# ruiguo-bio/smer_music_generation

Hardware: AMD Instinct MI355X
Metric: infill tokens/sec + train tokens/sec, SMER seq_len=1024, 1/2/4/8 MI355X (higher is better)
Workload: dtype bf16; 1 GPU; C2 train step: 6+6 layers d512 h8 ff2048 V309, per-GPU B=32 S=1024 T=256, dropout 0.1, fused WCE + Adam; global_batch=32, seq_len=1024, tgt_len=256, parallelism=dp1

## Files before the change

include/smer_hip.h:

```cpp
#ifndef SMER_HIP_H
#define SMER_HIP_H

#include <stddef.h>
#include <stdint.h>

#ifdef __cplusplus
extern "C" {
#endif

typedef struct ihipStream_t* smer_stream_t;

#define SMER_OK 0
#define SMER_ERR_INVALID (-1)
#define SMER_ERR_HIP (-2)
#define SMER_ERR_UNSUPPORTED (-3)

#define SMER_F32 0
#define SMER_BF16 1

int smer_abi_version(void);
const char* smer_last_error(void);

int smer_gemm(int dtype, int a_kcontig, int b_kcontig, int M, int N, int K,
              const void* A, long lda, const void* B, long ldb,
              const float* bias, float alpha, int relu,
              const void* residual, long ldr,
              const void* gate, long ldg, float gate_scale,
              float drop_p, uint32_t drop_seed,
              void* C, long ldc, float* Cf, long ldcf, int accumulate,
              void* workspace, size_t ws_bytes, smer_stream_t stream);

int smer_gemm_wgrad_bias(int dtype, int M, int N, int K, const void* dy, long lddy,
                         const void* x, long ldx, float* dW, long lddw, int accumulate,
                         float* db, int db_accumulate, void* workspace, size_t ws_bytes,
                         smer_stream_t stream);
int smer_gemm_wgrad_bias_ex(int dtype, int M, int N, int K, const void* dy, long lddy,
                            const void* x, long ldx, float* dW, long lddw, int accumulate,
                            float* db, int db_accumulate, void* workspace, size_t ws_bytes,
                            int max_workgroups, smer_stream_t stream);
int smer_gemm_wgrad_fp8(int M, int N, int K, const void* dy8, long lddy, const void* x8, long ldx,
                        const float* dy_inv, const float* x_inv, float* dW, long lddw, int accumulate,
                        float* db, int db_accumulate, void* workspace, size_t ws_bytes,
                        int max_workgroups, smer_stream_t stream);

int smer_gemm_debug_stamps(void* buf, size_t bytes);

int smer_attn_drop_mask_gen(int B, int H, int Lq, int Lk, float drop_p, uint32_t seed, void* mask,
                            smer_stream_t stream);
int smer_attn_fwd(int dtype, int B, int H, int Lq, int Lk, int D,
                  const void* q, long ldq, const void* k, long ldk, const void* v, long ldv,
                  void* o, long ldo, float* lse, const uint8_t* kpm, int causal, float scale,
                  float drop_p, uint32_t seed, void* drop_mask, int drop_mask_in,
                  smer_stream_t stream);
size_t smer_attn_drop_mask_bytes(int B, int H, int Lq, int Lk);
size_t smer_attn_bwd_workspace(int dtype, int B, int H, int Lq, int Lk);
int smer_attn_bwd(int dtype, int B, int H, int Lq, int Lk, int D,
                  const void* q, long ldq, const void* k, long ldk, const void* v, long ldv,
                  const void* o, long ldo, const void* dout, long lddo, const float* lse,
                  const uint8_t* kpm, int causal, float scale, float drop_p, uint32_t seed,
                  void* dq, long lddq, void* dk, long lddk, void* dv, long lddv,
                  void* workspace, size_t ws_bytes, const void* drop_mask,
                  smer_stream_t stream);
int smer_attn_bwd_fp8(int B, int H, int Lq, int Lk, int D, const void* q, long ldq,
                      const void* k, long ldk, const void* v, long ldv, const void* o, long ldo,
                      const void* dout, long lddo, const float* lse, const uint8_t* kpm,
                      int causal, float scale, float drop_p, uint32_t seed, void* dq, long lddq,
                      void* dk, long lddk, void* dv, long lddv, void* workspace, size_t ws_bytes,
                      const void* drop_mask, void* dq8, long lddq8, void* dk8, long lddk8,
                      void* dv8, long lddv8, const float* qs, unsigned* amax, smer_stream_t stream);
int smer_attn_fwd_fp8(int B, int H, int Lq, int Lk, int D, const void* q, long ldq, const void* k,
                      long ldk, const void* v, long ldv, void* o, long ldo, float* lse,
                      const uint8_t* kpm, int causal, float scale, float drop_p, uint32_t seed,
                      void* drop_mask, int drop_mask_in, void* o8, long ldo8, const float* qs,
                      unsigned* amax, smer_stream_t stream);
int smer_attn_weights(int dtype, int B, int H, int Lq, int Lk, int D,
                      const void* q, long ldq, const void* k, long ldk, const float* lse,
                      const uint8_t* kpm, int causal, float scale, float* out,
                      smer_stream_t stream);
int smer_attn_decode(int dtype, int n_rows, int H, int D, const void* q, long ldq,
                     const void* kcache, const void* vcache, long row_stride, long req_stride,
                     long head_stride, const int32_t* row_req, const int32_t* row_nkeys,
                     void* o, long ldo, float scale, smer_stream_t stream);
int smer_kv_scatter_heads(int dtype, int n_rows, int H, int D, const void* src, long lds,
                          void* cache, long req_stride, long kv_stride, long head_stride,
                          const int32_t* row_req, const int32_t* row_pos, smer_stream_t stream);
int smer_kv_scatter(int dtype, int n_rows, int width, const void* src, long lds,
                    void* cache, long row_stride, long req_stride,
                    const int32_t* row_req, const int32_t* row_pos, smer_stream_t stream);
int smer_linear_decode(int M, int N, int K, const void* A, long lda, const void* W, long ldw,
                       const float* bias, int relu, const void* residual, long ldr, void* C,
                       long ldc, float* Cf, long ldcf, void* kv, long kv_row_stride,
                       long kv_req_stride, const int32_t* kv_req, const int32_t* kv_pos,
                       int kv_col0, smer_stream_t stream);
int smer_attn_decode_qln(int n_rows, int H, int D, const void* y, long ldy, const float* gamma,
                         const float* beta, float eps, const void* wq, long ldw, const float* bq,
                         void* x_out, long ldx, int dmodel, const void* kcache, const void* vcache,
                         long row_stride, long req_stride, long head_stride, const int32_t* row_req,
                         const int32_t* row_nkeys, void* o, long ldo, float scale,
                         smer_stream_t stream);
int smer_attn_decode_shared(int dtype, int n_rows, int H, int D, const void* q, long ldq,
                            const void* kcache, const void* vcache, long row_stride,
                            long req_stride, long head_stride, const int32_t* row_req,
                            const int32_t* row_nkeys, const int32_t* group_tab, int n_groups,
                            void* o, long ldo, float scale, smer_stream_t stream);
int smer_attn_decode_shared_qln(int n_rows, int H, int D, const void* y, long ldy,
                                const float* gamma, const float* beta, float eps, const void* wq,
                                long ldw, const float* bq, void* x_out, long ldx, int dmodel,
                                const void* kcache, const void* vcache, long row_stride,
                                long req_stride, long head_stride, const int32_t* row_req,
                                const int32_t* row_nkeys, const int32_t* group_tab, int n_groups,
                                void* o, long ldo, float scale, smer_stream_t stream);
int smer_linear_decode_ln(int M, int N, int K, const void* Y, long ldy, const float* gamma,
                          const float* beta, float eps, void* X, long ldx, const void* W, long ldw,
                          const float* bias, int relu, const void* residual, long ldr, void* C,
                          long ldc, float* Cf, long ldcf, void* kv, long kv_row_stride,
                          long kv_req_stride, const int32_t* kv_req, const int32_t* kv_pos,
                          int kv_col0, smer_stream_t stream);
int smer_linear_decode_f32(int M, int N, int K, const void* A, long lda, const void* W, long ldw,
                           const float* bias, int relu, const void* residual, long ldr, void* C,
                           long ldc, float* Cf, long ldcf, void* kv, long kv_row_stride,
                           long kv_req_stride, const int32_t* kv_req, const int32_t* kv_pos,
                           int kv_col0, smer_stream_t stream);
int smer_linear_decode_ln_f32(int M, int N, int K, const void* Y, long ldy, const float* gamma,
                              const float* beta, float eps, void* X, long ldx, const void* W,
                              long ldw, const float* bias, int relu, const void* residual,
                              long ldr, void* C, long ldc, float* Cf, long ldcf, void* kv,
                              long kv_row_stride, long kv_req_stride, const int32_t* kv_req,
                              const int32_t* kv_pos, int kv_col0, smer_stream_t stream);
int smer_attn_decode_split_f32(int n_rows, int H, int D, const void* q, long ldq, const void* kcache,
                               const void* vcache, long row_stride, long req_stride, long head_stride,
                               const int32_t* row_req, const int32_t* row_nkeys, float* part, float scale,
                               smer_stream_t stream);
int smer_attn_decode_split_qln_f32(int n_rows, int H, int D, const float* y, long ldy, const float* gamma,
                                   const float* beta, float eps, const float* wq, long ldw, const float* bq,
                                   float* x_out, long ldx, int dmodel, const void* kcache, const void* vcache,
                                   long row_stride, long req_stride, long head_stride, const int32_t* row_req,
                                   const int32_t* row_nkeys, float* part, float scale, smer_stream_t stream);
int smer_linear_decode_merge_f32(int M, int N, int K, const float* part, const void* W, long ldw,
                                 const float* bias, int relu, const void* residual, long ldr, void* C,
                                 long ldc, float* Cf, long ldcf, smer_stream_t stream);
int smer_grammar_greedy_step(int R, int V, const float* logits, long ldl, int32_t* state,
                             int nst, const int8_t* targets, int max_masks, const uint8_t* keep,
                             const uint8_t* cls, int eos, int m0, int trash_pos, int max_span,
                             const int32_t* src_len, int64_t* ids, int32_t* meta,
                             int32_t* out_tok, int cap, int32_t* alive, smer_stream_t stream);
int smer_grammar_greedy_step_ring(int R, int V, const float* logits, long ldl, int32_t* state,
                                  int nst, const int8_t* targets, int max_masks,
                                  const uint8_t* keep, const uint8_t* cls, int eos, int m0,
                                  int trash_pos, int max_span, const int32_t* src_len,
                                  int64_t* ids, int32_t* meta, int32_t* out_tok, int cap,
                                  int32_t* ctl, int32_t* ring, int ring_n, smer_stream_t stream);
int smer_grammar_sample_step(int R, int V, const float* logits, long ldl, int32_t* state, int nst,
                             const int8_t* targets, int max_masks, const uint8_t* keep,
                             const uint8_t* reject, const uint8_t* cls, int eos, int m0,
                             int trash_pos, int max_span, const int32_t* src_len, int64_t* ids,
                             int32_t* meta, int32_t* out_tok, int cap, uint32_t* mt, int32_t* ctl,
                             int32_t* ring, int ring_n, smer_stream_t stream);
int smer_grammar_sample_step_tp(int R, int V, const float* logits, long ldl, int32_t* state, int nst,
                                const int8_t* targets, int max_masks, const uint8_t* keep,
                                const uint8_t* reject, const uint8_t* cls, int eos, int m0,
                                int trash_pos, int max_span, const int32_t* src_len, int64_t* ids,
                                int32_t* meta, int32_t* out_tok, int cap, uint32_t* mt, int32_t* ctl,
                                int32_t* ring, int ring_n, const double* tp, smer_stream_t stream);
int smer_grammar_sample_step_rows(int R, int V, const float* logits, long ldl, int32_t* state, int nst,
                                  const int8_t* targets, int max_masks, const uint8_t* keep,
                                  const uint8_t* reject, const uint8_t* cls, int eos, int m0,
                                  int trash_pos, int max_span, const int32_t* src_len, int64_t* ids,
                                  int32_t* meta, int32_t* out_tok, int cap, uint32_t* mt, long ldmt,
                                  int32_t* ctl, int32_t* ring, int ring_n, const double* tp,
                                  smer_stream_t stream);

int smer_layernorm_fwd(int dtype, int M, int N, const void* x, long ldx,
                       const float* gamma, const float* beta, float eps,
                       void* y, long ldy, float* mean, float* rstd, smer_stream_t stream);
size_t smer_layernorm_bwd_workspace(int M, int N);
int smer_layernorm_bwd(int dtype, int M, int N, const void* dy, long lddy, int dy_f32,
                       const void* x, long ldx, const float* mean, const float* rstd,
                       const float* gamma, void* dx, long lddx,
                       void* dx_drop, long ldxd, float drop_p, uint32_t seed,
                       float* dgamma, float* dbeta, int accumulate,
                       void* workspace, size_t ws_bytes, smer_stream_t stream);
int smer_layernorm_bwd_partials(int dtype, int M, int N, const void* dy, long lddy, int dy_f32,
                                const void* x, long ldx, const float* mean, const float* rstd,
                                const float* gamma, void* dx, long lddx, void* dx_drop,
                                long ldxd, float drop_p, uint32_t seed, void* workspace,
                                size_t ws_bytes, smer_stream_t stream);
int smer_layernorm_param_reduce(int M, int N, void* workspace, size_t ws_bytes, float* dgamma,
                                float* dbeta, int accumulate, smer_stream_t stream);

int smer_embed_fwd(int dtype, int n_tok, int d, const int64_t* ids, const int32_t* positions,
                   int L, const float* table, const float* pe, float scale,
                   float drop_p, uint32_t seed, void* out, long ldo, smer_stream_t stream);
int smer_embed_fwd_fp8(int n_tok, int d, const int64_t* ids, const int32_t* positions, int L,
                       const float* table, const float* pe, float scale, float drop_p, uint32_t seed,
                       void* out, long ldo, void* q8, long ldq, const float* qs, unsigned* amax,
                       smer_stream_t stream);
size_t smer_embed_bwd_workspace(int V, int d, int n_tok_total);
int smer_embed_bwd(int dtype, int V, int d, float scale,
                   const int64_t* ids0, const void* dx0, long ld0, int n0, float p0, uint32_t seed0,
                   const int64_t* ids1, const void* dx1, long ld1, int n1, float p1, uint32_t seed1,
                   float* dtable, void* workspace, size_t ws_bytes, smer_stream_t stream);

int smer_wce_denom(int n, const int64_t* y, const float* ce_all, float* denom,
                   smer_stream_t stream);
int smer_wce_fwd_bwd(int dtype, int R, int V, const float* logits, long ldl, const int64_t* y,
                     const float* w, const float* denom, float* row_loss, float* loss_out,
                     void* dlogits, long ldd, float grad_scale, smer_stream_t stream);

int smer_adam(long n, float* p, const float* g, float* m, float* v, void* p_bf16,
              float lr, float b1, float b2, float eps, float bc1, float bc2_sqrt,
              smer_stream_t stream);

int smer_cast(int src_dtype, int dst_dtype, long n, const void* src, void* dst,
              smer_stream_t stream);
int smer_cast2d(int src_dtype, int dst_dtype, int rows, int cols, const void* src, long lds,
                void* dst, long ldd, smer_stream_t stream);
int smer_debug_checksum(const void* p, long rows, long row_bytes, long ld_bytes,
                        unsigned long long* out, int nparts, smer_stream_t stream);
int smer_argmax_accuracy(int R, int V, const float* logits, long ldl, const int64_t* y,
                         const int32_t* cls, int ncls, int pad, unsigned* counts,
                         smer_stream_t stream);
size_t smer_colsum_workspace(int M, int N);
int smer_colsum(int dtype, int M, int N, const void* x, long ldx, float* out, int accumulate,
                void* workspace, size_t ws_bytes, smer_stream_t stream);

size_t smer_fp8_quantize_workspace(void);
int smer_fp8_quantize(int rows, int cols, const void* x, long ldx, void* q, long ldq,
                      void* workspace, float* inv_scale, smer_stream_t stream);
int smer_fp8_quantize_segments(int nseg, const int64_t* seg, unsigned* amax_ws, float* inv_scale,
                               int blocks_per_seg, smer_stream_t stream);
int smer_gemm_fp8(int M, int N, int K, const void* A, long lda, const void* B, long ldb,
                  const float* a_inv, const float* b_inv, const float* bias, int relu,
                  const void* residual, long ldr, float drop_p, uint32_t drop_seed, void* C,
                  long ldc, smer_stream_t stream);

int smer_gemm_fp8_q(int M, int N, int K, const void* A, long lda, const void* B, long ldb,
                    const float* a_inv, const float* b_inv, const float* bias, int relu,
                    const void* residual, long ldr, float drop_p, uint32_t drop_seed, void* C,
                    long ldc, void* q8, long ldq8, const float* qs, unsigned* amax,
                    smer_stream_t stream);
int smer_layernorm_fwd_fp8(int M, int N, const void* x, long ldx, const float* gamma,
                           const float* beta, float eps, void* y, long ldy, float* mean,
                           float* rstd, void* q8, long ldq, const float* qs, unsigned* amax,
                           smer_stream_t stream);
int smer_fp8_scales(int n, const unsigned* amax_prev, float* qs, float* inv, unsigned* amax_next,
                    smer_stream_t stream);

int smer_fp8_quantize_segments_t(int nseg, const int64_t* seg, unsigned* amax_ws, float* inv_scale,
                                 int blocks_per_seg, smer_stream_t stream);
int smer_gemm_fp8_ex(int M, int N, int K, const void* A, long lda, const void* B, long ldb,
                     const float* a_inv, const float* b_inv, const float* bias, int relu,
                     const void* residual, long ldr, const void* gate, long ldg, float gate_scale,
                     float drop_p, uint32_t drop_seed, void* C, long ldc, void* q8, long ldq8,
                     const float* qs, unsigned* amax, smer_stream_t stream);
int smer_gemm_fp8_gate8(int M, int N, int K, const void* A, long lda, const void* B, long ldb,
                        const float* a_inv, const float* b_inv, const void* gate8, long ldg,
                        float gate_scale, void* C, long ldc, void* q8, long ldq8, const float* q8_scale,
                        unsigned* q8_amax, smer_stream_t stream);
int smer_layernorm_bwd_fp8(int M, int N, const void* dy, long lddy, const void* x, long ldx,
                           const float* mean, const float* rstd, const float* gamma, void* dx,
                           long lddx, void* dx_drop, long ldxd, float drop_p, uint32_t seed,
                           void* q8, long ldq, const float* qs, unsigned* amax, float* dgamma,
                           float* dbeta, int accumulate, void* workspace, size_t ws_bytes,
                           int partials_only, smer_stream_t stream);

#ifdef __cplusplus
}
#endif
#endif
```

smer_music_generation_amd/_lib.py:

```python
from __future__ import annotations

import ctypes
import os

import torch

_HERE = os.path.dirname(os.path.abspath(__file__))
LIB_PATH = os.environ.get("SMER_HIP_LIB") or os.path.join(_HERE, "libsmer_hip.so")

c_int, c_long, c_float, c_size, c_u32 = (ctypes.c_int, ctypes.c_long, ctypes.c_float,
                                         ctypes.c_size_t, ctypes.c_uint32)
P = ctypes.c_void_p

SIGNATURES = {
    "smer_abi_version": (c_int, []),
    "smer_last_error": (ctypes.c_char_p, []),
    "smer_gemm": (c_int, [c_int, c_int, c_int, c_int, c_int, c_int, P, c_long, P, c_long, P,
                          c_float, c_int, P, c_long, P, c_long, c_float, c_float, c_u32, P,
                          c_long, P, c_long, c_int, P, c_size, P]),
    "smer_gemm_debug_stamps": (c_int, [P, c_size]),
    "smer_gemm_wgrad_bias": (c_int, [c_int, c_int, c_int, c_int, P, c_long, P, c_long, P, c_long,
                                     c_int, P, c_int, P, c_size, P]),
    "smer_embed_fwd_fp8": (c_int, [c_int, c_int, P, P, c_int, P, P, c_float, c_float, c_u32, P, c_long, P, c_long,
                                   P, P, P]),
    "smer_gemm_wgrad_fp8": (c_int, [c_int, c_int, c_int, P, c_long, P, c_long, P, P, P, c_long, c_int, P, c_int,
                                    P, c_size, c_int, P]),
    "smer_gemm_wgrad_bias_ex": (c_int, [c_int, c_int, c_int, c_int, P, c_long, P, c_long, P, c_long,
                                        c_int, P, c_int, P, c_size, c_int, P]),
    "smer_attn_fwd": (c_int, [c_int, c_int, c_int, c_int, c_int, c_int, P, c_long, P, c_long, P,
                              c_long, P, c_long, P, P, c_int, c_float, c_float, c_u32, P, c_int, P]),
    "smer_attn_fwd_fp8": (c_int, [c_int, c_int, c_int, c_int, c_int, P, c_long, P, c_long, P, c_long,
                                  P, c_long, P, P, c_int, c_float, c_float, c_u32, P, c_int, P, c_long,
                                  P, P, P]),
    "smer_attn_drop_mask_gen": (c_int, [c_int, c_int, c_int, c_int, c_float, c_u32, P, P]),
    "smer_attn_drop_mask_bytes": (c_size, [c_int, c_int, c_int, c_int]),
    "smer_attn_bwd_workspace": (c_size, [c_int, c_int, c_int, c_int, c_int]),
    "smer_attn_bwd": (c_int, [c_int, c_int, c_int, c_int, c_int, c_int, P, c_long, P, c_long, P,
                              c_long, P, c_long, P, c_long, P, P, c_int, c_float, c_float, c_u32,
                              P, c_long, P, c_long, P, c_long, P, c_size, P, P]),
    "smer_attn_bwd_fp8": (c_int, [c_int, c_int, c_int, c_int, c_int, P, c_long, P, c_long, P, c_long,
                                  P, c_long, P, c_long, P, P, c_int, c_float, c_float, c_u32, P, c_long,
                                  P, c_long, P, c_long, P, c_size, P, P, c_long, P, c_long, P, c_long,
                                  P, P, P]),
    "smer_attn_weights": (c_int, [c_int, c_int, c_int, c_int, c_int, c_int, P, c_long, P, c_long,
                                  P, P, c_int, c_float, P, P]),
    "smer_attn_decode": (c_int, [c_int, c_int, c_int, c_int, P, c_long, P, P, c_long, c_long,
                                 c_long, P, P, P, c_long, c_float, P]),
    "smer_attn_decode_qln": (c_int, [c_int, c_int, c_int, P, c_long, P, P, c_float, P, c_long, P,
                                     P, c_long, c_int, P, P, c_long, c_long, c_long, P, P, P, c_long,
                                     c_float, P]),
    "smer_attn_decode_shared": (c_int, [c_int, c_int, c_int, c_int, P, c_long, P, P, c_long, c_long,
                                        c_long, P, P, P, c_int, P, c_long, c_float, P]),
    "smer_attn_decode_shared_qln": (c_int, [c_int, c_int, c_int, P, c_long, P, P, c_float, P, c_long,
                                            P, P, c_long, c_int, P, P, c_long, c_long, c_long, P, P,
                                            P, c_int, P, c_long, c_float, P]),
    "smer_kv_scatter_heads": (c_int, [c_int, c_int, c_int, c_int, P, c_long, P, c_long, c_long,
                                      c_long, P, P, P]),
    "smer_kv_scatter": (c_int, [c_int, c_int, c_int, P, c_long, P, c_long, c_long, P, P, P]),
    "smer_linear_decode": (c_int, [c_int, c_int, c_int, P, c_long, P, c_long, P, c_int, P, c_long,
                                   P, c_long, P, c_long, P, c_long, c_long, P, P, c_int, P]),
    "smer_linear_decode_ln": (c_int, [c_int, c_int, c_int, P, c_long, P, P, c_float, P, c_long, P,
                                      c_long, P, c_int, P, c_long, P, c_long, P, c_long, P, c_long,
                                      c_long, P, P, c_int, P]),
    "smer_linear_decode_f32": (c_int, [c_int, c_int, c_int, P, c_long, P, c_long, P, c_int, P, c_long,
                                       P, c_long, P, c_long, P, c_long, c_long, P, P, c_int, P]),
    "smer_linear_decode_ln_f32": (c_int, [c_int, c_int, c_int, P, c_long, P, P, c_float, P, c_long, P,
                                          c_long, P, c_int, P, c_long, P, c_long, P, c_long, P, c_long,
                                          c_long, P, P, c_int, P]),
    "smer_attn_decode_split_f32": (c_int, [c_int, c_int, c_int, P, c_long, P, P, c_long, c_long, c_long, P, P, P,
                                           c_float, P]),
    "smer_attn_decode_split_qln_f32": (c_int, [c_int, c_int, c_int, P, c_long, P, P, c_float, P, c_long, P, P,
                                               c_long, c_int, P, P, c_long, c_long, c_long, P, P, P, c_float, P]),
    "smer_linear_decode_merge_f32": (c_int, [c_int, c_int, c_int, P, P, c_long, P, c_int, P, c_long, P, c_long, P,
                                             c_long, P]),
    "smer_fp8_quantize_workspace": (c_size, []),
    "smer_fp8_quantize": (c_int, [c_int, c_int, P, c_long, P, c_long, P, P, P]),
    "smer_fp8_quantize_segments": (c_int, [c_int, P, P, P, c_int, P]),
    "smer_gemm_fp8": (c_int, [c_int, c_int, c_int, P, c_long, P, c_long, P, P, P, c_int, P, c_long,
                              c_float, c_u32, P, c_long, P]),
    "smer_gemm_fp8_q": (c_int, [c_int, c_int, c_int, P, c_long, P, c_long, P, P, P, c_int, P,
                                c_long, c_float, c_u32, P, c_long, P, c_long, P, P, P]),
    "smer_layernorm_fwd_fp8": (c_int, [c_int, c_int, P, c_long, P, P, c_float, P, c_long, P, P, P,
                                       c_long, P, P, P]),
    "smer_fp8_scales": (c_int, [c_int, P, P, P, P, P]),
    "smer_fp8_quantize_segments_t": (c_int, [c_int, P, P, P, c_int, P]),
    "smer_gemm_fp8_ex": (c_int, [c_int, c_int, c_int, P, c_long, P, c_long, P, P, P, c_int, P, c_long,
                                 P, c_long, c_float, c_float, c_u32, P, c_long, P, c_long, P, P, P]),
    "smer_gemm_fp8_gate8": (c_int, [c_int, c_int, c_int, P, c_long, P, c_long, P, P, P, c_long, c_float,
                                    P, c_long, P, c_long, P, P, P]),
    "smer_layernorm_bwd_fp8": (c_int, [c_int, c_int, P, c_long, P, c_long, P, P, P, P, c_long, P, c_long,
                                       c_float, c_u32, P, c_long, P, P, P, P, c_int, P, c_size, c_int,
                                       P]),
    "smer_grammar_greedy_step": (c_int, [c_int, c_int, P, c_long, P, c_int, P, c_int, P, P, c_int,
                                         c_int, c_int, c_int, P, P, P, P, c_int, P, P]),
    "smer_grammar_greedy_step_ring": (c_int, [c_int, c_int, P, c_long, P, c_int, P, c_int, P, P,
                                              c_int, c_int, c_int, c_int, P, P, P, P, c_int, P, P,
                                              c_int, P]),
    "smer_grammar_sample_step": (c_int, [c_int, c_int, P, c_long, P, c_int, P, c_int, P, P, P,
                                         c_int, c_int, c_int, c_int, P, P, P, P, c_int, P, P, P,
                                         c_int, P]),
    "smer_grammar_sample_step_tp": (c_int, [c_int, c_int, P, c_long, P, c_int, P, c_int, P, P, P,
                                            c_int, c_int, c_int, c_int, P, P, P, P, c_int, P, P, P,
                                            c_int, P, P]),
    "smer_grammar_sample_step_rows": (c_int, [c_int, c_int, P, c_long, P, c_int, P, c_int, P, P, P,
                                              c_int, c_int, c_int, c_int, P, P, P, P, c_int, P, c_long,
                                              P, P, c_int, P, P]),
    "smer_layernorm_fwd": (c_int, [c_int, c_int, c_int, P, c_long, P, P, c_float, P, c_long, P,
                                   P, P]),
    "smer_layernorm_bwd_workspace": (c_size, [c_int, c_int]),
    "smer_layernorm_bwd": (c_int, [c_int, c_int, c_int, P, c_long, c_int, P, c_long, P, P, P, P,
                                   c_long, P, c_long, c_float, c_u32, P, P, c_int, P, c_size, P]),
    "smer_layernorm_bwd_partials": (c_int, [c_int, c_int, c_int, P, c_long, c_int, P, c_long, P, P,
                                            P, P, c_long, P, c_long, c_float, c_u32, P, c_size, P]),
    "smer_layernorm_param_reduce": (c_int, [c_int, c_int, P, c_size, P, P, c_int, P]),
    "smer_embed_fwd": (c_int, [c_int, c_int, c_int, P, P, c_int, P, P, c_float, c_float, c_u32,
                               P, c_long, P]),
    "smer_embed_bwd_workspace": (c_size, [c_int, c_int, c_int]),
    "smer_embed_bwd": (c_int, [c_int, c_int, c_int, c_float, P, P, c_long, c_int, c_float, c_u32,
                               P, P, c_long, c_int, c_float, c_u32, P, P, c_size, P]),
    "smer_wce_denom": (c_int, [c_int, P, P, P, P]),
    "smer_wce_fwd_bwd": (c_int, [c_int, c_int, c_int, P, c_long, P, P, P, P, P, P, c_long,
                                 c_float, P]),
    "smer_adam": (c_int, [c_long, P, P, P, P, P, c_float, c_float, c_float, c_float, c_float,
                          c_float, P]),
    "smer_cast": (c_int, [c_int, c_int, c_long, P, P, P]),
    "smer_cast2d": (c_int, [c_int, c_int, c_int, c_int, P, c_long, P, c_long, P]),
    "smer_colsum_workspace": (c_size, [c_int, c_int]),
    "smer_colsum": (c_int, [c_int, c_int, c_int, P, c_long, P, c_int, P, c_size, P]),
    "smer_debug_checksum": (c_int, [P, c_long, c_long, c_long, P, c_int, P]),
    "smer_argmax_accuracy": (c_int, [c_int, c_int, P, c_long, P, P, c_int, c_int, P, P]),
}

_lib = None
_load_error = None


def load():
    global _lib, _load_error
    if _lib is not None:
        return _lib
    if not os.path.exists(LIB_PATH):
        _load_error = "libsmer_hip.so not built (%s); run __graft_entry__.build()" % LIB_PATH
        raise RuntimeError(_load_error)
    lib = ctypes.CDLL(LIB_PATH, mode=ctypes.RTLD_GLOBAL)
    for name, (res, args) in SIGNATURES.items():
        fn = getattr(lib, name)
        fn.restype = res
        fn.argtypes = args
    _lib = lib
    return lib


class SmerError(RuntimeError):
    pass


def check(status, what):
    if status != 0:
        msg = load().smer_last_error()
        raise SmerError("%s failed (%d): %s" % (what, status, msg.decode() if msg else ""))


def call(name, *args):
    lib = load()
    check(getattr(lib, name)(*args), name)
```

smer_music_generation_amd/csrc/common.h:

```cpp
#pragma once
#include <hip/hip_runtime.h>
#include <stdint.h>

#include "../../include/smer_hip.h"

typedef __bf16 bf16;
typedef __bf16 bf16x8 __attribute__((ext_vector_type(8)));
typedef __bf16 bf16x4 __attribute__((ext_vector_type(4)));
typedef short i16x4 __attribute__((ext_vector_type(4)));
typedef float f32x4 __attribute__((ext_vector_type(4)));

#define SMER_WAVE 64

extern "C" int smer_set_error(int code, const char* msg);
#define SMER_CHECK_LAUNCH(what)                                          \
  do {                                                                   \
    hipError_t _e = hipGetLastError();                                   \
    if (_e != hipSuccess) return smer_set_error(SMER_ERR_HIP, hipGetErrorString(_e)); \
  } while (0)
#define SMER_REQUIRE(cond, msg) \
  do { if (!(cond)) return smer_set_error(SMER_ERR_INVALID, msg); } while (0)

template <typename T> __device__ __forceinline__ float to_f32(T x);
template <> __device__ __forceinline__ float to_f32<float>(float x) { return x; }
// ... 11 lines not shown
    case 0x141: return __int_as_float(__builtin_amdgcn_mov_dpp(__float_as_int(v), 0x141, 0xF, 0xF, false));
    default: return __int_as_float(__builtin_amdgcn_mov_dpp(__float_as_int(v), 0x140, 0xF, 0xF, false));
  }
}
template <typename OP>
__device__ __forceinline__ float wave_reduce(float v, OP op) {
  v = op(v, dpp_f(v, 0xB1));
  v = op(v, dpp_f(v, 0x4E));
  v = op(v, dpp_f(v, 0x141));
  v = op(v, dpp_f(v, 0x140));
  const auto a = __builtin_amdgcn_permlane16_swap(__float_as_uint(v), __float_as_uint(v), false, false);
  v = op(__uint_as_float(a[0]), __uint_as_float(a[1]));
  const auto b = __builtin_amdgcn_permlane32_swap(__float_as_uint(v), __float_as_uint(v), false, false);
  return op(__uint_as_float(b[0]), __uint_as_float(b[1]));
}
__device__ __forceinline__ float wave_sum(float v) {
  return wave_reduce(v, [](float x, float y) { return x + y; });
}
__device__ __forceinline__ float wave_max(float v) {
  return wave_reduce(v, [](float x, float y) { return fmaxf(x, y); });
}

__device__ __forceinline__ uint32_t smer_mix32(uint32_t h) {
  h ^= h >> 16; h *= 0x7FEB352Du; h ^= h >> 15; h *= 0x846CA68Bu; h ^= h >> 16;
  return h;
}
__device__ __forceinline__ uint32_t smer_rowkey(uint32_t seed, uint32_t row) {
  return smer_mix32(smer_mix32(row ^ 0x85EBCA6Bu) ^ seed);
}
__device__ __forceinline__ uint32_t smer_pair_bits(uint32_t rowkey, uint32_t pair) {
  return smer_mix32(rowkey + pair * 0x9E3779B9u);
}
__device__ __forceinline__ bool smer_keep16(uint32_t rowkey, uint32_t thr16, uint32_t col) {
  const uint32_t h = smer_pair_bits(rowkey, col >> 1);
  return ((col & 1u) ? (h >> 16) : (h & 0xFFFFu)) >= thr16;
}
__device__ __forceinline__ void smer_drop8(uint32_t rowkey, uint32_t thr16, float ds, uint32_t col0,
                                           float (&v)[8]) {
#pragma unroll
  for (int k = 0; k < 4; ++k) {
    const uint32_t h = smer_pair_bits(rowkey, (col0 >> 1) + k);
    v[2 * k] = (h & 0xFFFFu) >= thr16 ? v[2 * k] * ds : 0.f;
    v[2 * k + 1] = (h >> 16) >= thr16 ? v[2 * k + 1] * ds : 0.f;
  }
}
static inline uint32_t smer_drop_thr16(float p) {
  if (p <= 0.f) return 0u;
  long t = (long)((double)p * 65536.0 + 0.5);
  return (uint32_t)(t < 1 ? 1 : (t > 65535 ? 65535 : t));
}
static inline float smer_drop_scale16(uint32_t thr16) {
  return thr16 ? (float)(65536.0 / (65536.0 - (double)thr16)) : 1.f;
}

__device__ __forceinline__ uint32_t smer_attn_bits(uint32_t rowkey, uint32_t quad) {
  uint32_t h = rowkey + quad * 0x9E3779B9u;
  h ^= h >> 16;
  h = __umul24(h, 0xEB352Du);
  h ^= h >> 15;
  h = __umul24(h, 0x6CA68Bu);
  h ^= h >> 16;
  return h;
}
__device__ __forceinline__ uint32_t smer_attn_ge(uint32_t h, uint32_t lo4) {
  return (h | 0x80808080u) - lo4;
}
__device__ __forceinline__ bool smer_attn_keep(uint32_t rowkey, uint32_t thr7, uint32_t key) {
  return ((smer_attn_bits(rowkey, key >> 2) >> (8 * (key & 3))) & 0x7Fu) >= thr7;
}
static inline uint32_t smer_attn_thr7(float p) {
  if (p <= 0.f) return 0u;
  long t = (long)((double)p * 128.0 + 0.5);
  return (uint32_t)(t < 1 ? 1 : (t > 127 ? 127 : t));
}
static inline float smer_attn_scale7(uint32_t thr7) {
  return thr7 ? (float)(128.0 / (128.0 - (double)thr7)) : 1.f;
}

size_t smer_col_reduce_scratch(int nblk, int N);
void smer_col_reduce_launch(int nblk, int N, const float* part, long stride, long off, float* out,
                            int accumulate, float scale, float* scratch, hipStream_t s,
                            float* out2 = nullptr, int nsplit = 0);

template <typename T, bool VEC = true>
__device__ __forceinline__ void load8(const T* p, int valid, float (&v)[8]) {
  if (VEC && valid >= 8) {
    if constexpr (sizeof(T) == 2) {
      bf16x8 r = *reinterpret_cast<const bf16x8*>(p);
#pragma unroll
      for (int i = 0; i < 8; ++i) v[i] = (float)r[i];
    } else {
      float4 a = *reinterpret_cast<const float4*>(p), b = *reinterpret_cast<const float4*>(p + 4);
      v[0] = a.x; v[1] = a.y; v[2] = a.z; v[3] = a.w; v[4] = b.x; v[5] = b.y; v[6] = b.z; v[7] = b.w;
    }
  } else {
#pragma unroll
    for (int i = 0; i < 8; ++i) v[i] = i < valid ? (float)p[i] : 0.f;
  }
}

constexpr int LNR_MAXC = 4;
template <int NC = LNR_MAXC>
__device__ __forceinline__ void ln_stats_loaded(const float (&v)[NC][8], int N, float eps, int lane, float& mu,
                                                float& rs) {
  const int nch = N >> 3;
  float s = 0.f;
#pragma unroll
  for (int c = 0; c < NC; ++c)
    if (lane + 64 * c < nch)
#pragma unroll
      for (int i = 0; i < 8; ++i) s += v[c][i];
  mu = wave_sum(s) / N;
  float q = 0.f;
#pragma unroll
  for (int c = 0; c < NC; ++c)
    if (lane + 64 * c < nch)
#pragma unroll
      for (int i = 0; i < 8; ++i) {
        const float d = v[c][i] - mu;
        q += d * d;
      }
  rs = rsqrtf(wave_sum(q) / N + eps);
}
template <typename T, int NC = LNR_MAXC>
__device__ __forceinline__ void ln_row_stats(const T* __restrict__ xr, int N, float eps, int lane,
                                             float (&v)[NC][8], float& mu, float& rs) {
  const int nch = N >> 3;
  float s = 0.f;
#pragma unroll
  for (int c = 0; c < NC; ++c) {
    const int ch = lane + 64 * c;
    if (ch < nch) {
      load8<T>(xr + ch * 8, 8, v[c]);
#pragma unroll
      for (int i = 0; i < 8; ++i) s += v[c][i];
    }
  }
  mu = wave_sum(s) / N;
  float q = 0.f;
#pragma unroll
  for (int c = 0; c < NC; ++c)
    if (lane + 64 * c < nch)
#pragma unroll
      for (int i = 0; i < 8; ++i) {
        const float d = v[c][i] - mu;
        q += d * d;
      }
  rs = rsqrtf(wave_sum(q) / N + eps);
}
__device__ __forceinline__ float ln_apply(float v, float mu, float rs, float g, float b) {
  return __builtin_fmaf((v - mu) * rs, g, b);
}

__device__ __forceinline__ void xcd_block2d(int& bx, int& by) {
  const int nx = gridDim.x, n = gridDim.x * gridDim.y;
  const int b = blockIdx.y * nx + blockIdx.x;
  const int xcd = b & 7, q = n >> 3, r = n & 7;
  const int lin = (xcd < r ? xcd * (q + 1) : r * (q + 1) + (xcd - r) * q) + (b >> 3);
  bx = lin % nx;
  by = lin / nx;
}

__device__ __forceinline__ bf16x8 lds_read_b128(const char* base, uint32_t byte_off) {
  return *reinterpret_cast<const bf16x8*>(base + byte_off);
}
__device__ __forceinline__ bf16x4 lds_read_tr16(const char* base, uint32_t byte_off) {
// ... 107 lines not shown
```

smer_music_generation_amd/csrc/gemm.hip:

```cpp
#include "common.h"

#include <algorithm>
#include <cstdlib>

struct GemmEpi {
  const float* bias;
  float alpha;
  int relu;
  const void* residual;
  long ldr;
  const void* gate;
  long ldg;
  float gate_scale;
  uint32_t drop_thr;
  uint32_t seed;
  float drop_scale;
  void* C;
  long ldc;
  float* Cf;
  long ldcf;
  int accumulate;
  int vec;
  int rs_accumulate;
  void* kv;
// ... 1695 lines not shown
  e2.alpha = 1.f; e2.bias = nullptr; e2.relu = 0; e2.drop_thr = 0; e2.residual = nullptr;
  epi_apply8(e2, row + 1, col + 8, row, col, v);
}

template <int NW, int UNR, int MI = 4, bool KF = false>
__global__ __launch_bounds__(64 * NW) void gemm_skinny_bf16_kernel(int M, int N, int K,
                                                                   const bf16* __restrict__ A, long lda,
                                                                   const bf16* __restrict__ B, long ldb,
                                                                   GemmEpi e) {
  constexpr int BM = 16 * MI;
  __shared__ float red[NW][BM][SK_BN + 1];
  const int tid = threadIdx.x, lane = tid & 63, wave = tid >> 6;
  const int n0 = blockIdx.x * SK_BN, m0 = blockIdx.y * BM;
  const int r16 = lane & 15, kq = (lane >> 4) * 8;
  const int ncol = n0 + r16;
  const bool colok = ncol < N;
  const int erow = m0 + (tid >> 1), ecol = n0 + (tid & 1) * 8;
  const bool eth = tid < BM * 2;
  const bool pre = eth && epi_pre_ok(e, M, N, erow, ecol);
  EpiPre ep;
  if (!KF && pre) epi_prefetch(e, erow, ecol, ep);
  const bf16* bp = B + (long)(KF ? min(ncol, N - 1) : (colok ? ncol : 0)) * ldb + kq;
  const bf16* ap[MI];
  bool rowok[MI];
#pragma unroll
  for (int i = 0; i < MI; ++i) {
    const int row = m0 + i * 16 + r16;
    rowok[i] = row < M;
    ap[i] = A + (long)(KF ? min(row, M - 1) : (rowok[i] ? row : 0)) * lda + kq;
  }
  f32x4 acc[MI];
#pragma unroll
  for (int i = 0; i < MI; ++i) acc[i] = f32x4{0.f, 0.f, 0.f, 0.f};
  const int nsteps = (K + 31) / 32;
  for (int s0 = wave; s0 < nsteps; s0 += NW * UNR) {
    bf16x8 a[UNR][MI], b[UNR];
#pragma unroll
    for (int u = 0; u < UNR; ++u) {
      if constexpr (KF) {
        const int k = min(s0 + u * NW, nsteps - 1) * 32;
        b[u] = *reinterpret_cast<const bf16x8*>(bp + k);
#pragma unroll
        for (int i = 0; i < MI; ++i) a[u][i] = *reinterpret_cast<const bf16x8*>(ap[i] + k);
      } else {
        const int k = (s0 + u * NW) * 32;
        const bool kok = k + kq < K;
        b[u] = (colok && kok) ? *reinterpret_cast<const bf16x8*>(bp + k) : bf16x8{};
#pragma unroll
        for (int i = 0; i < MI; ++i)
          a[u][i] = (rowok[i] && kok) ? *reinterpret_cast<const bf16x8*>(ap[i] + k) : bf16x8{};
      }
    }
    if (KF && s0 == wave) epi_prefetch_clamped(e, M, N, erow, ecol, ep);
#pragma unroll
    for (int u = 0; u < UNR; ++u)
      if (!KF || s0 + u * NW < nsteps)
#pragma unroll
        for (int i = 0; i < MI; ++i) acc[i] = mfma16(a[u][i], b[u], acc[i]);
  }
  if (KF && wave >= nsteps) epi_prefetch_clamped(e, M, N, erow, ecol, ep);
  const int g = lane >> 4;
#pragma unroll
  for (int i = 0; i < MI; ++i)
#pragma unroll
    for (int r = 0; r < 4; ++r) red[wave][i * 16 + 4 * g + r][r16] = acc[i][r];
  __syncthreads();
  if (eth) {
    const int row = tid >> 1, ch = tid & 1;
    if (erow < M && ecol < N) {
      float v[8];
#pragma unroll
      for (int c = 0; c < 8; ++c) {
        float t = 0.f;
#pragma unroll
        for (int w = 0; w < NW; ++w) t += red[w][row][ch * 8 + c];
        v[c] = t;
      }
      if (pre) epi_apply8_pre(e, erow, ecol, v, ep);
      else epi_apply8(e, M, N, erow, ecol, v);
    }
  }
}

__global__ void splitk_reduce_kernel(int M, int N, int ksplit, const float* __restrict__ slabs,
                                     float alpha, float* __restrict__ Cf, long ldcf,
                                     int accumulate, const float* __restrict__ rs_part,
                                     float* __restrict__ rs_out, int rs_accumulate) {
  long idx = ((long)blockIdx.x * blockDim.x + threadIdx.x) * 4;
  long MN = (long)M * N;
  if (idx >= MN) {
    const long m = ((long)blockIdx.x * blockDim.x + threadIdx.x) - MN / 4;
    if (rs_out == nullptr || m >= M) return;
    float t = 0.f;
    for (int s = 0; s < ksplit; ++s) t += rs_part[(long)s * M + m];
    rs_out[m] = (rs_accumulate ? rs_out[m] : 0.f) + alpha * t;
    return;
  }
  float4 a = *reinterpret_cast<const float4*>(slabs + idx);
  int s = 1;
  for (; s + 4 <= ksplit; s += 4) {
    float4 b[4];
#pragma unroll
    for (int u = 0; u < 4; ++u) b[u] = *reinterpret_cast<const float4*>(slabs + (long)(s + u) * MN + idx);
#pragma unroll
    for (int u = 0; u < 4; ++u) {
      a.x += b[u].x; a.y += b[u].y; a.z += b[u].z; a.w += b[u].w;
    }
  }
  for (; s < ksplit; ++s) {
    float4 b = *reinterpret_cast<const float4*>(slabs + (long)s * MN + idx);
    a.x += b.x; a.y += b.y; a.z += b.z; a.w += b.w;
  }
  float v[4] = {a.x * alpha, a.y * alpha, a.z * alpha, a.w * alpha};
  if ((N & 3) == 0 && (ldcf & 3) == 0 && (((uintptr_t)Cf) & 15) == 0) {
    const long row = idx / N;
    float* p = Cf + row * ldcf + (idx - row * N);
    float4 o = make_float4(v[0], v[1], v[2], v[3]);
    if (accumulate) {
      const float4 c = *reinterpret_cast<const float4*>(p);
      o.x = c.x + o.x; o.y = c.y + o.y; o.z = c.z + o.z; o.w = c.w + o.w;
    }
    *reinterpret_cast<float4*>(p) = o;
    return;
  }
#pragma unroll
  for (int t = 0; t < 4; ++t) {
    long e = idx + t;
    int row = e / N, col = e % N;
    float* p = Cf + (long)row * ldcf + col;
    *p = accumulate ? *p + v[t] : v[t];
  }
}

template <bool AK, bool BKC>
__global__ __launch_bounds__(256) void gemm_f32_kernel(int M, int N, int K,
                                                       const float* __restrict__ A, long lda,
                                                       const float* __restrict__ B, long ldb,
                                                       GemmEpi e) {
  __shared__ float As[16][68];
  __shared__ float Bs[16][68];
  const int tid = threadIdx.x, tx = tid & 15, ty = tid >> 4;
  const int m0 = blockIdx.y * 64, n0 = blockIdx.x * 64;
  float acc[4][4] = {};
  for (int k0 = 0; k0 < K; k0 += 16) {
#pragma unroll
    for (int c = 0; c < 4; ++c) {
      int i = tid + 256 * c;
      int m, kk;
      if (AK) { m = i >> 4; kk = i & 15; } else { kk = i >> 6; m = i & 63; }
      int gm = m0 + m, gk = k0 + kk;
      float a = 0.f;
      if (gm < M && gk < K) a = AK ? A[(long)gm * lda + gk] : A[(long)gk * lda + gm];
      As[kk][m] = a;
      int n;
      if (BKC) { n = i >> 4; kk = i & 15; } else { kk = i >> 6; n = i & 63; }
      int gn = n0 + n;
      gk = k0 + kk;
      float b = 0.f;
      if (gn < N && gk < K) b = BKC ? B[(long)gn * ldb + gk] : B[(long)gk * ldb + gn];
      Bs[kk][n] = b;
    }
    __syncthreads();
#pragma unroll
    for (int kk = 0; kk < 16; ++kk) {
      float a[4], b[4];
#pragma unroll
      for (int i = 0; i < 4; ++i) a[i] = As[kk][ty * 4 + i];
#pragma unroll
      for (int j = 0; j < 4; ++j) b[j] = Bs[kk][tx * 4 + j];
#pragma unroll
      for (int i = 0; i < 4; ++i)
#pragma unroll
        for (int j = 0; j < 4; ++j) acc[i][j] = fmaf(a[i], b[j], acc[i][j]);
    }
    __syncthreads();
  }
#pragma unroll
  for (int i = 0; i < 4; ++i)
#pragma unroll
    for (int j = 0; j < 4; ++j)
      epi_apply<float>(e, M, N, m0 + ty * 4 + i, n0 + tx * 4 + j, acc[i][j]);
}

static bool smer_gemm_glds_enabled() {
  static int v = -1;
  if (v < 0) {
    const char* e = getenv("SMER_GEMM_GLDS");
    v = (e && e[0] == '0') ? 0 : 1;
  }
  return v == 1;
}

static bool smer_wgrad_glds() {
  static int v = -1;
  if (v < 0) {
    const char* e = getenv("SMER_WGRAD_GLDS");
    v = (e && e[0] == '0') ? 0 : 1;
  }
  return v == 1;
}

static bool smer_gemm256_enabled() {
  const char* e = getenv("SMER_GEMM256");
  return !(e && e[0] == '0');
}

static bool smer_gemm256s_enabled(bool bkc, int N, int K) {
  const char* e = getenv("SMER_GEMM256S");
  if (e && e[0] == '1') return true;
  if (e && e[0] == '0') return false;
  return K >= 1024 || (!bkc && N >= 1024);
}

// ... 57 lines not shown
  }
  return wgrad_cap(v);
}
static int smer_wgrad256_depth() {
  static int v = -1;
  if (v < 0) {
    const char* e = getenv("SMER_WGRAD256_DEPTH");
    v = e ? std::max(64, atoi(e)) : 512;
  }
  return v;
}

static bool smer_skinny16_enabled() {
  static int v = -1;
  if (v < 0) {
    const char* e = getenv("SMER_SKINNY16");
    v = (e && e[0] == '0') ? 0 : 1;
  }
  return v == 1;
}

static long smer_skinny16_cap() {
  static int v = -1;
  if (v < 0) {
    const char* e = getenv("SMER_SKINNY16_CAP");
    v = e ? std::max(1, atoi(e)) : 2;
  }
  return v;
}

static int smer_wgrad_stages() {
  static int v = -1;
  if (v < 0) {
    const char* e = getenv("SMER_WGRAD_STAGES");
    v = e ? std::max(2, std::min(4, atoi(e))) : 2;
  }
  return v;
}
static size_t smer_wgrad_lds_pad() {
  static long v = -1;
  if (v < 0) {
    const char* e = getenv("SMER_WGRAD_LDS_PAD");
    v = e ? std::max(0, std::min(96 * 1024, atoi(e))) : 0;
  }
  return (size_t)v;
}
static long smer_wgrad_resident() {
  static int v = -1;
  if (v < 0) {
    const char* e = getenv("SMER_WGRAD_WGP2");
    v = e ? std::max(1, std::min(4, atoi(e))) : 4;
  }
  return wgrad_cap(std::max(8L, (v * (long)smer_num_cus()) / 2));
}

static long smer_g256_min_tiles() {
  static long v = -1;
  if (v < 0) {
    const char* e = getenv("SMER_G256_MIN");
    v = e ? std::max(1, atoi(e)) : smer_num_cus();
  }
  return v;
}

constexpr size_t SPLITK_TICKET_BYTES = 64 * 1024;
static bool smer_splitk_fused() {
  const char* e = getenv("SMER_SPLITK_FUSED");
  return e && e[0] == '1';
}
static size_t splitk_slab_bytes(size_t ws_bytes) {
  return ws_bytes > SPLITK_TICKET_BYTES ? ws_bytes - SPLITK_TICKET_BYTES : 0;
}

static int choose_split(int M, int N, int K, const GemmEpi& e, size_t ws_bytes) {
  bool cf_only = e.Cf && !e.C && !e.bias && !e.residual && !e.gate && !e.relu && !e.drop_thr;
  if (!cf_only) return 1;
  long tiles = (long)((M + GBM - 1) / GBM) * ((N + GBN - 1) / GBN);
  if (tiles >= 512 || K < 1024 || ((long)M * N) % 4 != 0) return 1;
  long s = smer_wgrad_resident() / tiles;
  s = std::min<long>(s, K / smer_splitk_depth());
  s = std::min<long>(s, (long)(splitk_slab_bytes(ws_bytes) / (((size_t)M * N + M) * sizeof(float))));
  s = std::max<long>(1, std::min<long>(s, 64));
  return (int)s;
}

static bool smer_skinny_kf() {
  static int v = -1;
  if (v < 0) {
    const char* e = getenv("SMER_SKINNY_KF");
    v = (e && e[0] == '0') ? 0 : 1;
  }
  return v == 1;
}

template <bool AK, bool BKC>
static void launch_bf16(int M, int N, int K, const void* A, long lda, const void* B, long ldb,
                        const GemmEpi& e, void* ws, size_t ws_bytes, hipStream_t s,
                        float* rowsum = nullptr) {
  if (AK && BKC && M <= 4 * SK_BM && !rowsum) {
    const int nsteps = (K + 31) / 32;
    const int ntn = (N + SK_BN - 1) / SK_BN;
    const bool m16 = smer_skinny16_enabled() && (long)ntn * ((M + 15) / 16) <= smer_skinny16_cap() * smer_num_cus();
    const bool kf = K % 32 == 0 && smer_skinny_kf();
#define SKB(U, MI)                                                                                     \
  do {                                                                                                 \
    if (kf)                                                                                            \
      hipLaunchKernelGGL((gemm_skinny_bf16_kernel<8, U, MI, true>), grid, dim3(512), 0, s, M, N, K,    \
                         (const bf16*)A, lda, (const bf16*)B, ldb, e);                                 \
    else                                                                                               \
      hipLaunchKernelGGL((gemm_skinny_bf16_kernel<8, U, MI, false>), grid, dim3(512), 0, s, M, N, K,   \
                         (const bf16*)A, lda, (const bf16*)B, ldb, e);                                 \
  } while (0)
    if (m16) {
      const dim3 grid(ntn, (M + 15) / 16);
      if (nsteps > 16) SKB(4, 1);
      else SKB(2, 1);
      return;
    }
    const dim3 grid(ntn, (M + SK_BM - 1) / SK_BM);
    if (nsteps > 16) SKB(4, 4);
    else SKB(2, 4);
#undef SKB
    return;
  }
  if (AK && !rowsum && K % G2K == 0 && smer_gemm256_enabled()) {
    const long t2 = (long)((M + G2 - 1) / G2) * ((N + G2 - 1) / G2);
    if (t2 >= smer_g256_min_tiles() && smer_gemm256s_enabled(BKC, N, K) && M % G2 == 0 && N % G2 == 0 &&
        K % GS_KS == 0 && K / GS_KS >= 4 && e.vec && e.C && !e.Cf && !e.kv && !e.q8 &&
        !(e.residual && e.gate)) {
      static bool attr_s = false;
      if (!attr_s) {
        hipFuncSetAttribute((const void*)gemm256s_bf16_kernel<true>,
                            hipFuncAttributeMaxDynamicSharedMemorySize, G2_LDS);
        hipFuncSetAttribute((const void*)gemm256s_bf16_kernel<false>,
                            hipFuncAttributeMaxDynamicSharedMemorySize, G2_LDS);
        attr_s = true;
      }
      const int np = smer_g256_nonpersist();
      const bool whole = np == 2 || (np == 1 && !BKC);
      const int grid = (t2 > smer_num_cus() && !whole) ? (smer_num_cus() & ~7) : (int)t2;
      GemmEpi ed = e;
      ed.dbg = gemm_dbg_for(grid, s);
      ed.skew = smer_g256_skew();
      hipLaunchKernelGGL(gemm256s_bf16_kernel<BKC>, dim3(grid), dim3(512), G2_LDS, s,
                         M, N, K, (const bf16*)A, lda, (const bf16*)B, ldb, ed);
      return;
    }
    if (t2 >= smer_g256_min_tiles()) {
      const int np = smer_g256_nonpersist();
      const bool whole = np == 2 || (np == 1 && !BKC);
      const int grid = (t2 > smer_num_cus() && !whole) ? (smer_num_cus() & ~7) : (int)t2;
      static bool attr_set = false;
      if (!attr_set) {
        hipFuncSetAttribute((const void*)gemm256_bf16_kernel<AK, BKC, false>,
                            hipFuncAttributeMaxDynamicSharedMemorySize, G2_LDS);
        hipFuncSetAttribute((const void*)gemm256_bf16_kernel<AK, BKC, true>,
                            hipFuncAttributeMaxDynamicSharedMemorySize, G2_LDS);
        attr_set = true;
      }
      const bool fast = e.vec && e.C && !e.Cf && !e.kv && M % G2 == 0 && N % G2 == 0 &&
                        !(e.residual && e.gate);
      auto kern = fast ? gemm256_bf16_kernel<AK, BKC, true> : gemm256_bf16_kernel<AK, BKC, false>;
      GemmEpi ek = e;
      ek.skew = smer_g256_skew();
      hipLaunchKernelGGL(kern, dim3(grid), dim3(512), G2_LDS, s,
                         M, N, K, (const bf16*)A, lda, (const bf16*)B, ldb, ek);
      return;
    }
  }
  if (!AK && !BKC && K % G2K == 0 && ws && smer_wgrad256_enabled(M, N)) {
    const bool cf_only = e.Cf && !e.C && !e.bias && !e.residual && !e.gate && !e.relu && !e.drop_thr &&
                         ((long)M * N) % 4 == 0;
    const long t2 = (long)((M + G2 - 1) / G2) * ((N + G2 - 1) / G2);
    const long cus = smer_num_cus();
    long ns = std::min<long>(smer_wgrad256_slots() / std::max<long>(1, t2), K / smer_wgrad256_depth());
    ns = std::min<long>(ns, (long)(splitk_slab_bytes(ws_bytes) / (((size_t)M * N + M) * sizeof(float))));
    ns = std::max<long>(1, std::min<long>(ns, 64));
    if (cf_only && t2 * ns * 4 >= 3 * cus) {
      int kchunk = (int)(((K + ns - 1) / ns + G2K - 1) / G2K * G2K);
      const int split = (K + kchunk - 1) / kchunk;
      static bool attr_set = false;
      if (!attr_set) {
        hipFuncSetAttribute((const void*)gemm256_wgrad_kernel, hipFuncAttributeMaxDynamicSharedMemorySize,
                            2 * G2_STAGE);
        attr_set = true;
      }
      float* rs_part = (split > 1 && rowsum) ? (float*)ws + (size_t)split * M * N : nullptr;
      const long nwg = t2 * split;
      const long gcap = wgrad_cap(cus);
      const int grid = nwg > gcap ? (int)(gcap & ~7L) : (int)nwg;
      if (smer_wgrad256s_enabled() && M % G2 == 0 && N % G2 == 0 && e.vec) {
        static bool attr_s = false;
        if (!attr_s) {
          hipFuncSetAttribute((const void*)gemm256s_wgrad_kernel, hipFuncAttributeMaxDynamicSharedMemorySize,
                              4 * GS_SLOT);
          attr_s = true;
        }
        hipLaunchKernelGGL(gemm256s_wgrad_kernel, dim3(grid), dim3(512), 4 * GS_SLOT, s, M, N, K,
                           (const bf16*)A, lda, (const bf16*)B, ldb, e, split, kchunk, (float*)ws,
                           split > 1 ? rs_part : rowsum);
      } else
      hipLaunchKernelGGL(gemm256_wgrad_kernel, dim3(grid), dim3(512), 2 * G2_STAGE, s, M, N, K,
                         (const bf16*)A, lda, (const bf16*)B, ldb, e, split, kchunk, (float*)ws,
                         split > 1 ? rs_part : rowsum);
      if (split > 1) {
        long n4 = ((long)M * N) / 4 + (rowsum ? M : 0);
        hipLaunchKernelGGL(splitk_reduce_kernel, dim3((n4 + 255) / 256), dim3(256), 0, s, M, N, split,
                           (const float*)ws, e.alpha, e.Cf, e.ldcf, e.accumulate,
                           (const float*)rs_part, rowsum, e.rs_accumulate);
      }
      return;
    }
  }
  int tiles = ((M + GBM - 1) / GBM) * ((N + GBN - 1) / GBN);
  int split = choose_split(M, N, K, e, ws ? ws_bytes : 0);
  if (AK && !rowsum && split == 1 && K % GBK == 0 && tiles <= 4 * smer_num_cus() &&
      M > 4 * SK_BM && smer_gemm_glds_enabled() && smer_gemm64_enabled()) {
    const long t64 = (long)((M + 63) / 64) * ((N + GBN - 1) / GBN);
    const long res = 3L * smer_num_cus();
    const int grid = t64 > res ? (int)(res & ~7L) : (int)t64;
    hipLaunchKernelGGL((gemm64_bf16_kernel<BKC>), dim3(grid), dim3(256), 2 * G64_STAGE, s, M, N, K,
                       (const bf16*)A, lda, (const bf16*)B, ldb, e);
    return;
  }
  int kchunk = K;
  if (split > 1) {
    kchunk = ((K + split - 1) / split + GBK - 1) / GBK * GBK;
    split = (K + kchunk - 1) / kchunk;
  }
  float* rs_part = (split > 1 && rowsum) ? (float*)ws + (size_t)split * M * N : nullptr;
  unsigned* tickets = nullptr;
  if (split > 1 && smer_splitk_fused() && (N & 3) == 0 && (e.ldcf & 3) == 0 &&
      ((uintptr_t)e.Cf & 15) == 0 && (size_t)tiles * 4 <= SPLITK_TICKET_BYTES &&
      ws_bytes >= SPLITK_TICKET_BYTES)
    tickets = (unsigned*)((char*)ws + ws_bytes - SPLITK_TICKET_BYTES);
  const long nwg = (long)tiles * split;
  const long resident = split > 1 ? smer_wgrad_resident() : 2L * smer_num_cus();
  const int grid = nwg > resident ? (int)(resident & ~7L) : (int)nwg;
  const bool gl = (K % GBK) == 0 && (kchunk % GBK) == 0 && smer_gemm_glds_enabled() &&
                  ((AK || BKC) || smer_wgrad_glds());
  if constexpr (!AK && !BKC) {
    const int ns = smer_wgrad_stages();
    if (gl && split > 1 && smer_wgrad_resident() <= smer_num_cus() && ns > 2) {
      static bool attr = false;
      if (!attr) {
        hipFuncSetAttribute((const void*)gemm_bf16_kernel<false, false, true, 3>,
                            hipFuncAttributeMaxDynamicSharedMemorySize, 6 * TILE_BYTES);
        hipFuncSetAttribute((const void*)gemm_bf16_kernel<false, false, true, 4>,
                            hipFuncAttributeMaxDynamicSharedMemorySize, 8 * TILE_BYTES);
        attr = true;
      }
      if (ns == 4)
        hipLaunchKernelGGL((gemm_bf16_kernel<false, false, true, 4>), dim3(grid), dim3(256), 8 * TILE_BYTES, s,
                           M, N, K, (const bf16*)A, lda, (const bf16*)B, ldb, e, split, kchunk, (float*)ws,
                           rs_part, tickets, rowsum);
      else
        hipLaunchKernelGGL((gemm_bf16_kernel<false, false, true, 3>), dim3(grid), dim3(256), 6 * TILE_BYTES, s,
                           M, N, K, (const bf16*)A, lda, (const bf16*)B, ldb, e, split, kchunk, (float*)ws,
                           rs_part, tickets, rowsum);
      goto reduce;
    }
  }
  {
    auto kern = gl ? gemm_bf16_kernel<AK, BKC, true> : gemm_bf16_kernel<AK, BKC, false>;
    size_t lds = 4 * TILE_BYTES;
    if (!AK && !BKC && gl && smer_wgrad_lds_pad()) {
      lds += smer_wgrad_lds_pad();
      static bool attr_pad = false;
      if (!attr_pad) {
        hipFuncSetAttribute((const void*)gemm_bf16_kernel<false, false, true>,
                            hipFuncAttributeMaxDynamicSharedMemorySize, 160 * 1024);
        attr_pad = true;
      }
    }
    hipLaunchKernelGGL(kern, dim3(grid), dim3(256), lds,
                       s, M, N, K, (const bf16*)A, lda, (const bf16*)B, ldb, e, split, kchunk,
                       (float*)ws, split > 1 ? rs_part : rowsum, tickets, rowsum);
  }
reduce:
  if (split > 1 && !tickets) {
    long n4 = ((long)M * N) / 4 + (rowsum ? M : 0);
    hipLaunchKernelGGL(splitk_reduce_kernel, dim3((n4 + 255) / 256), dim3(256), 0, s, M, N, split,
                       (const float*)ws, e.alpha, e.Cf, e.ldcf, e.accumulate,
                       (const float*)rs_part, rowsum, e.rs_accumulate);
  }
}
constexpr int SKF_BN = 4, SKF_BM = 16, SKF_NW = 4, SKF_UNR = 8;
__global__ __launch_bounds__(64 * SKF_NW) void gemm_skinny_f32_kernel(int M, int N, int K,
                                                                      const float* __restrict__ A, long lda,
                                                                      const float* __restrict__ B, long ldb,
                                                                      GemmEpi e) {
  __shared__ float red[SKF_NW][SKF_BM][SKF_BN];
  const int tid = threadIdx.x, lane = tid & 63, wave = tid >> 6;
  const int cq = lane >> 4, kq = lane & 15;
  const int n0 = blockIdx.x * SKF_BN, m0 = blockIdx.y * SKF_BM;
  const int col = n0 + cq;
  const bool colok = col < N;
  const int mrows = min(SKF_BM, M - m0);
  const float* bp = B + (long)(colok ? col : 0) * ldb + 4 * kq;
  const float* a0 = A + (long)m0 * lda + 4 * kq;
  float acc[SKF_BM];
#pragma unroll
  for (int r = 0; r < SKF_BM; ++r) acc[r] = 0.f;
  const int nsteps = (K + 63) / 64;
  for (int s0 = wave; s0 < nsteps; s0 += SKF_NW * SKF_UNR) {
    float4 b[SKF_UNR];
#pragma unroll
    for (int u = 0; u < SKF_UNR; ++u) {
      const int k = (s0 + u * SKF_NW) * 64;
      b[u] = (colok && k + 4 * kq < K) ? *reinterpret_cast<const float4*>(bp + k) : make_float4(0, 0, 0, 0);
    }
#pragma unroll
    for (int u = 0; u < SKF_UNR; ++u) {
      const int k = (s0 + u * SKF_NW) * 64;
      if (k + 4 * kq >= K) continue;
#pragma unroll
      for (int r = 0; r < SKF_BM; ++r) {
        if (r < mrows) {
          const float4 a = *reinterpret_cast<const float4*>(a0 + (long)r * lda + k);
          acc[r] = fmaf(a.x, b[u].x, acc[r]);
          acc[r] = fmaf(a.y, b[u].y, acc[r]);
          acc[r] = fmaf(a.z, b[u].z, acc[r]);
          acc[r] = fmaf(a.w, b[u].w, acc[r]);
        }
      }
    }
  }
#pragma unroll
  for (int r = 0; r < SKF_BM; ++r) {
    if (r < mrows) {
      acc[r] += __shfl_xor(acc[r], 1, 64);
      acc[r] += __shfl_xor(acc[r], 2, 64);
      acc[r] += __shfl_xor(acc[r], 4, 64);
      acc[r] += __shfl_xor(acc[r], 8, 64);
    }
  }
  if (kq == 0) {
#pragma unroll
    for (int r = 0; r < SKF_BM; ++r) red[wave][r][cq] = acc[r];
  }
  __syncthreads();
  if (tid < SKF_BM * SKF_BN) {
    const int r = tid / SKF_BN, c = tid % SKF_BN;
    if (r < mrows && n0 + c < N) {
      float t = 0.f;
#pragma unroll
      for (int w = 0; w < SKF_NW; ++w) t += red[w][r][c];
      epi_apply<float>(e, M, N, m0 + r, n0 + c, t);
    }
  }
}

template <int PD>
__global__ __launch_bounds__(256) void gemm_f32_mfma_kernel(int M, int N, int K, const float* __restrict__ A,
                                                            long lda, const float* __restrict__ B, long ldb,
                                                            GemmEpi e) {
  const int lane = threadIdx.x & 63, wave = threadIdx.x >> 6;
  const int c16 = lane & 15, g = lane >> 4;
  const int m0 = blockIdx.y * 64 + (wave >> 1) * 32, n0 = blockIdx.x * 64 + (wave & 1) * 32;
  const float* ap[2];
  const float* bp[2];
#pragma unroll
  for (int i = 0; i < 2; ++i) {
    const int r = m0 + 16 * i + c16, c = n0 + 16 * i + c16;
// ... 77 lines not shown
    v = (e && e[0] == '0') ? 0 : 1;
  }
  return v == 1;
}
template <bool AK, bool BKC>
static void launch_f32(int M, int N, int K, const void* A, long lda, const void* B, long ldb,
                       const GemmEpi& e, hipStream_t s) {
  if (AK && BKC && M <= 64 && K % 4 == 0 && lda % 4 == 0 && ldb % 4 == 0 &&
      (((uintptr_t)A | (uintptr_t)B) & 15) == 0) {
    if (K <= SKF_NW * SKF_UNR * 64 && smer_skinny_rows_f32()) {
      launch_skinny_rows_f32(M, N, K, (const float*)A, lda, (const float*)B, ldb, e, s);
      return;
    }
    const dim3 grid((N + SKF_BN - 1) / SKF_BN, (M + SKF_BM - 1) / SKF_BM);
    hipLaunchKernelGGL(gemm_skinny_f32_kernel, grid, dim3(64 * SKF_NW), 0, s, M, N, K, (const float*)A,
                       lda, (const float*)B, ldb, e);
    return;
  }
  dim3 grid((N + 63) / 64, (M + 63) / 64);
  if (AK && BKC && K % 4 == 0 && lda % 4 == 0 && ldb % 4 == 0 &&
      (((uintptr_t)A | (uintptr_t)B) & 15) == 0 && smer_gemm_f32_mfma()) {
    hipLaunchKernelGGL(gemm_f32_mfma_kernel<2>, grid, dim3(256), 0, s, M, N, K, (const float*)A, lda,
                       (const float*)B, ldb, e);
    return;
  }
  hipLaunchKernelGGL((gemm_f32_kernel<AK, BKC>), grid, dim3(256), 0, s, M, N, K,
                     (const float*)A, lda, (const float*)B, ldb, e);
}

static bool aligned16(const void* p) { return ((uintptr_t)p & 15) == 0; }

extern "C" int smer_gemm(int dtype, int a_kcontig, int b_kcontig, int M, int N, int K,
                         const void* A, long lda, const void* B, long ldb, const float* bias,
                         float alpha, int relu, const void* residual, long ldr, const void* gate,
                         long ldg, float gate_scale, float drop_p, uint32_t drop_seed, void* C,
                         long ldc, float* Cf, long ldcf, int accumulate, void* workspace,
                         size_t ws_bytes, smer_stream_t stream) {
  SMER_REQUIRE(M >= 0 && N >= 0 && K >= 0, "smer_gemm: negative size");
  SMER_REQUIRE(A && B, "smer_gemm: null operand");
  SMER_REQUIRE(C || Cf, "smer_gemm: no output");
  SMER_REQUIRE(drop_p >= 0.f && drop_p < 1.f, "smer_gemm: drop_p out of range");
  if (M == 0 || N == 0) return SMER_OK;
  GemmEpi e{};
  e.bias = bias; e.alpha = alpha; e.relu = relu; e.residual = residual; e.ldr = ldr;
  e.gate = gate; e.ldg = ldg; e.gate_scale = gate_scale;
  e.drop_thr = smer_drop_thr16(drop_p); e.seed = drop_seed;
  e.drop_scale = smer_drop_scale16(e.drop_thr);
  e.C = C; e.ldc = ldc; e.Cf = Cf; e.ldcf = ldcf; e.accumulate = accumulate;
  e.rs_accumulate = 0;
  auto a16 = [](const void* p, long ld) { return p == nullptr || ((((uintptr_t)p) & 15) == 0 && ld % 8 == 0); };
  e.vec = a16(bias, 8) && a16(residual, ldr) && a16(gate, ldg) && a16(C, ldc) && a16(Cf, ldcf);
  hipStream_t s = (hipStream_t)stream;
  if (dtype == SMER_BF16) {
    SMER_REQUIRE(K % 8 == 0, "smer_gemm(bf16): K must be a multiple of 8");
    SMER_REQUIRE(lda % 8 == 0 && ldb % 8 == 0, "smer_gemm(bf16): lda/ldb must be multiples of 8");
    SMER_REQUIRE(aligned16(A) && aligned16(B), "smer_gemm(bf16): operands must be 16-B aligned");
    SMER_REQUIRE(a_kcontig || lda >= (long)((M + 7) / 8) * 8,
                 "smer_gemm(bf16): column-image A needs lda >= round_up(M, 8)");
    SMER_REQUIRE(b_kcontig || ldb >= (long)((N + 7) / 8) * 8,
                 "smer_gemm(bf16): column-image B needs ldb >= round_up(N, 8)");
    SMER_REQUIRE(!workspace || aligned16(workspace), "smer_gemm: workspace alignment");
    if (K == 0) return smer_set_error(SMER_ERR_UNSUPPORTED, "smer_gemm: K == 0");
    if (a_kcontig && b_kcontig) launch_bf16<true, true>(M, N, K, A, lda, B, ldb, e, workspace, ws_bytes, s);
    else if (a_kcontig) launch_bf16<true, false>(M, N, K, A, lda, B, ldb, e, workspace, ws_bytes, s);
    else if (b_kcontig) launch_bf16<false, true>(M, N, K, A, lda, B, ldb, e, workspace, ws_bytes, s);
    else launch_bf16<false, false>(M, N, K, A, lda, B, ldb, e, workspace, ws_bytes, s);
  } else if (dtype == SMER_F32) {
    if (a_kcontig && b_kcontig) launch_f32<true, true>(M, N, K, A, lda, B, ldb, e, s);
    else if (a_kcontig) launch_f32<true, false>(M, N, K, A, lda, B, ldb, e, s);
    else if (b_kcontig) launch_f32<false, true>(M, N, K, A, lda, B, ldb, e, s);
    else launch_f32<false, false>(M, N, K, A, lda, B, ldb, e, s);
  } else {
    return smer_set_error(SMER_ERR_UNSUPPORTED, "smer_gemm: dtype");
  }
  SMER_CHECK_LAUNCH("smer_gemm");
  return SMER_OK;
}

extern "C" int smer_gemm_wgrad_bias(int dtype, int M, int N, int K, const void* dy, long lddy,
                                    const void* x, long ldx, float* dW, long lddw, int accumulate,
                                    float* db, int db_accumulate, void* workspace,
                                    size_t ws_bytes, smer_stream_t stream) {
  return smer_gemm_wgrad_bias_ex(dtype, M, N, K, dy, lddy, x, ldx, dW, lddw, accumulate, db,
                                 db_accumulate, workspace, ws_bytes, 0, stream);
}

extern "C" int smer_gemm_wgrad_bias_ex(int dtype, int M, int N, int K, const void* dy, long lddy,
                                       const void* x, long ldx, float* dW, long lddw, int accumulate,
                                       float* db, int db_accumulate, void* workspace,
                                       size_t ws_bytes, int max_workgroups, smer_stream_t stream) {
  SMER_REQUIRE(dtype == SMER_BF16, "smer_gemm_wgrad_bias: bf16 only (fp32: smer_gemm + smer_colsum)");
  SMER_REQUIRE(M > 0 && N > 0 && K > 0, "smer_gemm_wgrad_bias: bad sizes");
  SMER_REQUIRE(dy && x && dW && db, "smer_gemm_wgrad_bias: null pointer");
  SMER_REQUIRE(lddy % 8 == 0 && ldx % 8 == 0 && lddy >= (long)((M + 7) / 8) * 8 &&
                   ldx >= (long)((N + 7) / 8) * 8,
               "smer_gemm_wgrad_bias: dy / x row strides");
  SMER_REQUIRE(aligned16(dy) && aligned16(x) && (!workspace || aligned16(workspace)),
               "smer_gemm_wgrad_bias: 16-B alignment");
  GemmEpi e{};
  e.alpha = 1.f; e.drop_scale = 1.f;
  e.Cf = dW; e.ldcf = lddw; e.accumulate = accumulate; e.rs_accumulate = db_accumulate;
  auto a16 = [](const void* p, long ld) { return p == nullptr || ((((uintptr_t)p) & 15) == 0 && ld % 8 == 0); };
  e.vec = a16(dW, lddw);
  g_wgrad_cap = max_workgroups > 0 ? max_workgroups : 0;
  launch_bf16<false, false>(M, N, K, dy, lddy, x, ldx, e, workspace, ws_bytes, (hipStream_t)stream, db);
  g_wgrad_cap = 0;
  SMER_CHECK_LAUNCH("smer_gemm_wgrad_bias");
  return SMER_OK;
}

template <int NW, int UNR, int NC = LNR_MAXC, bool KF = false>
__global__ __launch_bounds__(64 * NW) void gemm_skinny_ln_kernel(int M, int N, int K,
                                                                 const bf16* __restrict__ Y, long ldy,
                                                                 const float* __restrict__ gamma,
                                                                 const float* __restrict__ beta, float eps,
                                                                 bf16* __restrict__ X, long ldx,
                                                                 const bf16* __restrict__ B, long ldb,
                                                                 GemmEpi e) {
  constexpr int BM = 16;
  extern __shared__ __attribute__((aligned(16))) char xs[];
  __shared__ float red[NW][BM][SK_BN + 1];
  const int tid = threadIdx.x, lane = tid & 63, wave = tid >> 6;
  const int n0 = blockIdx.x * SK_BN, m0 = blockIdx.y * BM;
  const long xs_ld = 2L * K + 32;
  const int erow = m0 + (tid >> 1), ecol = n0 + (tid & 1) * 8;
  const bool eth = tid < BM * 2;
  const bool pre = eth && epi_pre_ok(e, M, N, erow, ecol);
  EpiPre ep;
  if (!KF && pre) epi_prefetch(e, erow, ecol, ep);
  const int r16 = lane & 15, kq = (lane >> 4) * 8;
  const int ncol = n0 + r16;
  const bool colok = ncol < N;
  const bf16* bp = B + (long)(KF ? min(ncol, N - 1) : (colok ? ncol : 0)) * ldb + kq;
  const int nsteps = (K + 31) / 32;
  bf16x8 b0[UNR];
#pragma unroll
  for (int u = 0; u < UNR; ++u) {
    const int k = (wave + u * NW) * 32;
    if constexpr (KF) b0[u] = *reinterpret_cast<const bf16x8*>(bp + min(k, (nsteps - 1) * 32));
    else b0[u] = (colok && k + kq < K) ? *reinterpret_cast<const bf16x8*>(bp + k) : bf16x8{};
  }
  const int nch = K >> 3;
  if constexpr (KF) {
    constexpr int RPW = BM / NW;
    bf16x8 yv[RPW][NC];
    float4 gv[NC][2], bv[NC][2];
#pragma unroll
    for (int j = 0; j < RPW; ++j) {
      const bf16* yr = Y + (long)min(m0 + wave + NW * j, M - 1) * ldy;
#pragma unroll
      for (int c = 0; c < NC; ++c) yv[j][c] = *reinterpret_cast<const bf16x8*>(yr + 8 * min(lane + 64 * c, nch - 1));
    }
#pragma unroll
    for (int c = 0; c < NC; ++c) {
      const int ch = min(lane + 64 * c, nch - 1);
      gv[c][0] = *reinterpret_cast<const float4*>(gamma + ch * 8);
      gv[c][1] = *reinterpret_cast<const float4*>(gamma + ch * 8 + 4);
      bv[c][0] = *reinterpret_cast<const float4*>(beta + ch * 8);
      bv[c][1] = *reinterpret_cast<const float4*>(beta + ch * 8 + 4);
    }
    epi_prefetch_clamped(e, M, N, erow, ecol, ep);
#pragma unroll
    for (int j = 0; j < RPW; ++j) {
      const int rr = wave + NW * j, row = m0 + rr;
      char* dst = xs + rr * xs_ld;
      float v[NC][8], mu, rs;
#pragma unroll
      for (int c = 0; c < NC; ++c)
#pragma unroll
        for (int i = 0; i < 8; ++i) v[c][i] = (float)yv[j][c][i];
      ln_stats_loaded<NC>(v, K, eps, lane, mu, rs);
#pragma unroll
      for (int c = 0; c < NC; ++c) {
        const int ch = lane + 64 * c;
        if (ch < nch) {
          const float g[8] = {gv[c][0].x, gv[c][0].y, gv[c][0].z, gv[c][0].w,
                              gv[c][1].x, gv[c][1].y, gv[c][1].z, gv[c][1].w};
          const float b[8] = {bv[c][0].x, bv[c][0].y, bv[c][0].z, bv[c][0].w,
                              bv[c][1].x, bv[c][1].y, bv[c][1].z, bv[c][1].w};
          bf16x8 o;
#pragma unroll
          for (int i = 0; i < 8; ++i) o[i] = (bf16)ln_apply(v[c][i], mu, rs, g[i], b[i]);
          *reinterpret_cast<bf16x8*>(dst + ch * 16) = o;
          if (X && blockIdx.x == 0 && row < M) *reinterpret_cast<bf16x8*>(X + (long)row * ldx + ch * 8) = o;
        }
      }
    }
  } else {
  for (int rr = wave; rr < BM; rr += NW) {
// ... 1492 lines not shown
```

smer_music_generation_amd/csrc/norm_embed.hip:

```cpp
#include "common.h"

namespace {
constexpr int LN_MAXC = 4;

template <typename T> struct Vec8;
template <> struct Vec8<bf16> {
  static __device__ __forceinline__ void load(const bf16* p, float (&v)[8]) {
    bf16x8 r = *reinterpret_cast<const bf16x8*>(p);
#pragma unroll
    for (int i = 0; i < 8; ++i) v[i] = (float)r[i];
  }
  static __device__ __forceinline__ void store(bf16* p, const float (&v)[8]) {
    bf16x8 r;
#pragma unroll
    for (int i = 0; i < 8; ++i) r[i] = (bf16)v[i];
    *reinterpret_cast<bf16x8*>(p) = r;
  }
};
template <> struct Vec8<float> {
  static __device__ __forceinline__ void load(const float* p, float (&v)[8]) {
    float4 a = *reinterpret_cast<const float4*>(p), b = *reinterpret_cast<const float4*>(p + 4);
    v[0] = a.x; v[1] = a.y; v[2] = a.z; v[3] = a.w; v[4] = b.x; v[5] = b.y; v[6] = b.z; v[7] = b.w;
  }
  static __device__ __forceinline__ void store(float* p, const float (&v)[8]) {
// ... 810 lines not shown
    if (ln_bwd_t4_rb(Q) == 2) LNBT4R(2, Q);              \
    else LNBT4R(4, Q);                                   \
  } while (0)
#define LNBQ(NC, RB, PF)                                                                                   \
  hipLaunchKernelGGL((ln_bwd_kernel<bf16, false, NC, RB, PF, true>), dim3(nblk), dim3(256), 0, s, M, N,    \
                     dy, lddy, (const bf16*)x, ldx, mean, rstd, gamma, (bf16*)dx, lddx, (bf16*)dx_drop,    \
                     ldxd, thr, seed, ds, part, rpb, q8, ldq, qs, amax)
#define LNBQ1(NC, RB)                                  \
  do {                                                 \
    if (rpb / 4 > (RB)) LNBQ(NC, RB, true);            \
    else LNBQ(NC, RB, false);                          \
  } while (0)
  if (q8) {
    if (t4) LNBT4(true);
    else if (N <= 512) LNBQ1(1, 4);
    else if (N <= 1024) LNBQ1(2, 2);
    else LNBQ1(4, 1);
  } else if (t4) {
    LNBT4(false);
  } else if (dtype == SMER_BF16) { if (dy_f32) LNB(bf16, true); else LNB(bf16, false); }
  else if (dtype == SMER_F32) { LNB(float, false); }
  else return smer_set_error(SMER_ERR_UNSUPPORTED, "smer_layernorm_bwd: dtype");
#undef LNB
#undef LNB1
#undef LNB2
#undef LNBT4
#undef LNBT4R
#undef LNBQ
#undef LNBQ1
  if (reduce) {
    if (dgamma && dbeta)
      smer_col_reduce_launch(nblk, 2 * N, part, (long)2 * N, 0L, dgamma, accumulate, 1.f,
                             part + (size_t)nblk * 2 * N, s, dbeta, N);
    else if (dgamma)
      smer_col_reduce_launch(nblk, N, part, (long)2 * N, 0L, dgamma, accumulate, 1.f,
                             part + (size_t)nblk * 2 * N, s);
    else if (dbeta)
      smer_col_reduce_launch(nblk, N, part, (long)2 * N, (long)N, dbeta, accumulate, 1.f,
                             part + (size_t)nblk * 2 * N, s);
  }
  SMER_CHECK_LAUNCH("smer_layernorm_bwd");
  return SMER_OK;
}

extern "C" int smer_layernorm_bwd(int dtype, int M, int N, const void* dy, long lddy, int dy_f32,
                                  const void* x, long ldx, const float* mean, const float* rstd,
                                  const float* gamma, void* dx, long lddx, void* dx_drop,
                                  long ldxd, float drop_p, uint32_t seed, float* dgamma,
                                  float* dbeta, int accumulate, void* workspace, size_t ws_bytes,
                                  smer_stream_t stream) {
  return ln_bwd_impl(dtype, M, N, dy, lddy, dy_f32, x, ldx, mean, rstd, gamma, dx, lddx, dx_drop,
                     ldxd, drop_p, seed, dgamma, dbeta, accumulate, workspace, ws_bytes, stream,
                     dgamma || dbeta, true);
}

extern "C" int smer_layernorm_bwd_partials(int dtype, int M, int N, const void* dy, long lddy,
                                           int dy_f32, const void* x, long ldx, const float* mean,
                                           const float* rstd, const float* gamma, void* dx,
                                           long lddx, void* dx_drop, long ldxd, float drop_p,
                                           uint32_t seed, void* workspace, size_t ws_bytes,
                                           smer_stream_t stream) {
  SMER_REQUIRE(workspace, "smer_layernorm_bwd_partials: workspace required");
  return ln_bwd_impl(dtype, M, N, dy, lddy, dy_f32, x, ldx, mean, rstd, gamma, dx, lddx, dx_drop,
                     ldxd, drop_p, seed, nullptr, nullptr, 0, workspace, ws_bytes, stream, true,
                     false);
}

extern "C" int smer_layernorm_bwd_fp8(int M, int N, const void* dy, long lddy, const void* x, long ldx,
                                      const float* mean, const float* rstd, const float* gamma, void* dx,
                                      long lddx, void* dx_drop, long ldxd, float drop_p, uint32_t seed,
                                      void* q8, long ldq, const float* qs, unsigned* amax, float* dgamma,
                                      float* dbeta, int accumulate, void* workspace, size_t ws_bytes,
                                      int partials_only, smer_stream_t stream) {
  SMER_REQUIRE(q8, "smer_layernorm_bwd_fp8: q8 required");
  SMER_REQUIRE(!partials_only || workspace, "smer_layernorm_bwd_fp8: partials need a workspace");
  const bool params = partials_only || dgamma || dbeta;
  return ln_bwd_impl(SMER_BF16, M, N, dy, lddy, 0, x, ldx, mean, rstd, gamma, dx, lddx, dx_drop, ldxd,
                     drop_p, seed, dgamma, dbeta, accumulate, workspace, ws_bytes, stream, params,
                     !partials_only, (uint8_t*)q8, ldq, qs, amax);
}

extern "C" int smer_layernorm_param_reduce(int M, int N, void* workspace, size_t ws_bytes,
                                           float* dgamma, float* dbeta, int accumulate,
                                           smer_stream_t stream) {
  SMER_REQUIRE(workspace && ws_bytes >= smer_layernorm_bwd_workspace(M, N),
               "smer_layernorm_param_reduce: workspace too small");
  if (M == 0 || (!dgamma && !dbeta)) return SMER_OK;
  const int nblk = (M + ln_bwd_rows(M, N) - 1) / ln_bwd_rows(M, N);
  float* part = (float*)workspace;
  hipStream_t s = (hipStream_t)stream;
  if (dgamma && dbeta)
    smer_col_reduce_launch(nblk, 2 * N, part, (long)2 * N, 0L, dgamma, accumulate, 1.f,
                           part + (size_t)nblk * 2 * N, s, dbeta, N);
  else if (dgamma)
    smer_col_reduce_launch(nblk, N, part, (long)2 * N, 0L, dgamma, accumulate, 1.f,
                           part + (size_t)nblk * 2 * N, s);
  else
    smer_col_reduce_launch(nblk, N, part, (long)2 * N, (long)N, dbeta, accumulate, 1.f,
                           part + (size_t)nblk * 2 * N, s);
  SMER_CHECK_LAUNCH("smer_layernorm_param_reduce");
  return SMER_OK;
}

extern "C" int smer_embed_fwd(int dtype, int n_tok, int d, const int64_t* ids,
                              const int32_t* positions, int L, const float* table,
                              const float* pe, float scale, float drop_p, uint32_t seed,
                              void* out, long ldo, smer_stream_t stream) {
  SMER_REQUIRE(d % 4 == 0, "smer_embed_fwd: d % 4 == 0");
  SMER_REQUIRE(positions || L > 0, "smer_embed_fwd: L");
  if (n_tok == 0) return SMER_OK;
  hipStream_t s = (hipStream_t)stream;
  long tot = (long)n_tok * (d / 4);
  uint32_t thr = smer_drop_thr16(drop_p);
  float ds = smer_drop_scale16(thr);
  if (dtype == SMER_BF16)
    hipLaunchKernelGGL(embed_fwd_kernel<bf16>, dim3((tot + 255) / 256), dim3(256), 0, s, n_tok, d,
                       ids, positions, L, table, pe, scale, thr, seed, ds, (bf16*)out, ldo);
  else if (dtype == SMER_F32)
    hipLaunchKernelGGL(embed_fwd_kernel<float>, dim3((tot + 255) / 256), dim3(256), 0, s, n_tok, d,
                       ids, positions, L, table, pe, scale, thr, seed, ds, (float*)out, ldo);
  else
    return smer_set_error(SMER_ERR_UNSUPPORTED, "smer_embed_fwd: dtype");
  SMER_CHECK_LAUNCH("smer_embed_fwd");
  return SMER_OK;
}

extern "C" int smer_embed_fwd_fp8(int n_tok, int d, const int64_t* ids, const int32_t* positions, int L,
                                  const float* table, const float* pe, float scale, float drop_p,
                                  uint32_t seed, void* out, long ldo, void* q8, long ldq, const float* qs,
                                  unsigned* amax, smer_stream_t stream) {
  SMER_REQUIRE(d % 4 == 0 && ldq % 4 == 0 && ((uintptr_t)q8 & 3) == 0, "smer_embed_fwd_fp8: d, ldq % 4 == 0");
  SMER_REQUIRE(positions || L > 0, "smer_embed_fwd_fp8: L");
  SMER_REQUIRE(ids && table && pe && out && q8 && qs && amax, "smer_embed_fwd_fp8: null pointer");
  if (n_tok == 0) return SMER_OK;
  hipStream_t s = (hipStream_t)stream;
  long tot = (long)n_tok * (d / 4);
  uint32_t thr = smer_drop_thr16(drop_p);
  float ds = smer_drop_scale16(thr);
  hipLaunchKernelGGL((embed_fwd_kernel<bf16, true>), dim3((tot + 255) / 256), dim3(256), 0, s, n_tok, d, ids,
                     positions, L, table, pe, scale, thr, seed, ds, (bf16*)out, ldo, (uint8_t*)q8, ldq, qs, amax);
  SMER_CHECK_LAUNCH("smer_embed_fwd_fp8");
  return SMER_OK;
}

extern "C" size_t smer_embed_bwd_workspace(int V, int d, int n_tok_total) {
  size_t nchunk = (size_t)(n_tok_total + EMB_CHUNK - 1) / EMB_CHUNK;
  if (nchunk == 0) nchunk = 1;
  return nchunk * V * d * sizeof(float);
}

extern "C" int smer_embed_bwd(int dtype, int V, int d, float scale, const int64_t* ids0,
                              const void* dx0, long ld0, int n0, float p0, uint32_t seed0,
                              const int64_t* ids1, const void* dx1, long ld1, int n1, float p1,
                              uint32_t seed1, float* dtable, void* workspace, size_t ws_bytes,
                              smer_stream_t stream) {
  SMER_REQUIRE(d % 64 == 0 && d <= 1024, "smer_embed_bwd: d % 64 == 0 and d <= 1024");
  SMER_REQUIRE((!dx0 || (ld0 % 8 == 0 && ((uintptr_t)dx0 & 15) == 0)) &&
                   (!dx1 || (ld1 % 8 == 0 && ((uintptr_t)dx1 & 15) == 0)),
               "smer_embed_bwd: dx rows must be 16-B aligned (ld % 8 == 0)");
  SMER_REQUIRE(workspace && ws_bytes >= smer_embed_bwd_workspace(V, d, n0 + n1),
               "smer_embed_bwd: workspace too small");
  int n = n0 + n1;
  if (n == 0) return SMER_OK;
  hipStream_t s = (hipStream_t)stream;
  int nchunk = (n + EMB_CHUNK - 1) / EMB_CHUNK;
  uint32_t t0 = smer_drop_thr16(p0), t1 = smer_drop_thr16(p1);
  float ds0 = smer_drop_scale16(t0), ds1 = smer_drop_scale16(t1);
  dim3 grid(V, nchunk);
  if (dtype == SMER_BF16)
    hipLaunchKernelGGL(embed_bwd_gather<bf16>, grid, dim3(256), 0, s, V, d, ids0, (const bf16*)dx0,
                       ld0, n0, t0, seed0, ds0, ids1, (const bf16*)dx1, ld1, n1, t1, seed1, ds1,
                       (float*)workspace);
  else if (dtype == SMER_F32)
// ... 12 lines not shown
```

smer_music_generation_amd/csrc/train_ops.hip:

```cpp
#include "common.h"

__global__ __launch_bounds__(256) void wce_denom_kernel(int n, const int64_t* __restrict__ y,
                                                        const float* __restrict__ ce_all,
                                                        float* __restrict__ denom) {
  __shared__ float red[256];
  float a = 0.f;
  for (int i = threadIdx.x; i < n; i += 256) a += ce_all[y[i]];
  red[threadIdx.x] = a;
  __syncthreads();
  for (int s = 128; s > 0; s >>= 1) {
    if (threadIdx.x < s) red[threadIdx.x] += red[threadIdx.x + s];
    __syncthreads();
  }
  if (threadIdx.x == 0) *denom = red[0];
}

template <typename T>
__global__ __launch_bounds__(256) void wce_kernel(int R, int V, const float* __restrict__ logits,
                                                  long ldl, const int64_t* __restrict__ y,
                                                  const float* __restrict__ w,
                                                  const float* __restrict__ denom,
                                                  float* __restrict__ row_loss,
                                                  T* __restrict__ dlog, long ldd,
                                                  float grad_scale) {
// ... 30 lines not shown
  red[threadIdx.x] = a;
  __syncthreads();
  for (int s = 128; s > 0; s >>= 1) {
    if (threadIdx.x < s) red[threadIdx.x] += red[threadIdx.x + s];
    __syncthreads();
  }
  if (threadIdx.x == 0) *out = denom ? red[0] / *denom : red[0];
}

__global__ void adam_kernel(long n, float* __restrict__ p, const float* __restrict__ g,
                            float* __restrict__ m, float* __restrict__ v, bf16* __restrict__ pb,
                            float lr, float b1, float b2, float eps, float bc1, float bc2s) {
  long i = (long)blockIdx.x * blockDim.x + threadIdx.x;
  const long stride = (long)gridDim.x * blockDim.x;
  const float step = lr / bc1;
  for (; i < n; i += stride) {
    float gi = g[i];
    float mi = m[i];
    mi = mi + (1.f - b1) * (gi - mi);
    float vi = v[i] * b2 + (1.f - b2) * gi * gi;
    float den = sqrtf(vi) / bc2s + eps;
    float pi = p[i] - step * (mi / den);
    m[i] = mi;
    v[i] = vi;
    p[i] = pi;
    if (pb) pb[i] = (bf16)pi;
  }
}

template <typename S, typename D>
__global__ void cast_kernel(long n, const S* __restrict__ s, D* __restrict__ d) {
  long i = (long)blockIdx.x * blockDim.x + threadIdx.x;
  const long stride = (long)gridDim.x * blockDim.x;
  for (; i < n; i += stride) d[i] = from_f32<D>(to_f32(s[i]));
}

constexpr int CS_ROWS = 64;
template <typename T, bool VEC>
__global__ __launch_bounds__(256) void colsum_part_kernel(int M, int N, const T* __restrict__ x,
                                                          long ldx, float* __restrict__ part) {
  __shared__ float red[4][512];
  const int cg = threadIdx.x & 63, rg = threadIdx.x >> 6;
  const int c0 = blockIdx.x * 512 + cg * 8;
  const int r0 = blockIdx.y * CS_ROWS;
  const int r1 = min(M, r0 + CS_ROWS);
  const int valid = min(8, N - c0);
  float acc[8] = {0.f, 0.f, 0.f, 0.f, 0.f, 0.f, 0.f, 0.f};
  if (valid > 0) {
    int r = r0 + rg;
    for (; r + 12 < r1; r += 16) {
      float v0[8], v1[8], v2[8], v3[8];
      load8<T, VEC>(x + (long)r * ldx + c0, valid, v0);
      load8<T, VEC>(x + (long)(r + 4) * ldx + c0, valid, v1);
      load8<T, VEC>(x + (long)(r + 8) * ldx + c0, valid, v2);
      load8<T, VEC>(x + (long)(r + 12) * ldx + c0, valid, v3);
#pragma unroll
      for (int i = 0; i < 8; ++i) acc[i] += (v0[i] + v1[i]) + (v2[i] + v3[i]);
    }
    for (; r < r1; r += 4) {
      float v0[8];
      load8<T, VEC>(x + (long)r * ldx + c0, valid, v0);
#pragma unroll
      for (int i = 0; i < 8; ++i) acc[i] += v0[i];
    }
  }
#pragma unroll
  for (int i = 0; i < 8; ++i) red[rg][cg * 8 + i] = acc[i];
  __syncthreads();
  for (int c = threadIdx.x; c < 512; c += 256) {
    int col = blockIdx.x * 512 + c;
    if (col < N) part[(long)blockIdx.y * N + col] = (red[0][c] + red[1][c]) + (red[2][c] + red[3][c]);
  }
}

__global__ void __launch_bounds__(256) smer_col_reduce(int nblk, int N, const float* __restrict__ part,
                                                       long stride, long off, float* __restrict__ out,
                                                       long ostride, int chunk, int accumulate,
                                                       float scale, float* __restrict__ out2,
                                                       int nsplit) {
  __shared__ float red[4][64];
  const int cl = threadIdx.x & 63, g = threadIdx.x >> 6;
  const int col = blockIdx.x * 64 + cl;
  const int b0 = blockIdx.y * chunk, b1 = min(nblk, b0 + chunk);
  float a0 = 0.f, a1 = 0.f, a2 = 0.f, a3 = 0.f;
  if (col < N) {
    const float* p = part + off + col;
    int b = b0 + g;
    for (; b + 12 < b1; b += 16) {
      a0 += p[(long)b * stride];
      a1 += p[(long)(b + 4) * stride];
      a2 += p[(long)(b + 8) * stride];
      a3 += p[(long)(b + 12) * stride];
    }
    for (; b < b1; b += 4) a0 += p[(long)b * stride];
  }
  red[g][cl] = (a0 + a1) + (a2 + a3);
  __syncthreads();
  if (g == 0 && col < N) {
    float a = ((red[0][cl] + red[1][cl]) + (red[2][cl] + red[3][cl])) * scale;
    float* o = col < nsplit ? out + (long)blockIdx.y * ostride + col
                            : out2 + (long)blockIdx.y * ostride + (col - nsplit);
    *o = accumulate ? *o + a : a;
  }
}

size_t smer_col_reduce_scratch(int nblk, int N) {
  return nblk > 64 ? (size_t)((nblk + 63) / 64) * N * sizeof(float) : 0;
}

void smer_col_reduce_launch(int nblk, int N, const float* part, long stride, long off, float* out,
                            int accumulate, float scale, float* scratch, hipStream_t s,
                            float* out2, int nsplit) {
  dim3 gx((N + 63) / 64);
  if (!out2) nsplit = N;
  if (nblk > 64) {
    int g = (nblk + 63) / 64;
    hipLaunchKernelGGL(smer_col_reduce, dim3(gx.x, g), dim3(256), 0, s, nblk, N, part, stride,
                       off, scratch, (long)N, 64, 0, 1.f, (float*)nullptr, N);
    hipLaunchKernelGGL(smer_col_reduce, dim3(gx.x, 1), dim3(256), 0, s, g, N,
                       (const float*)scratch, (long)N, 0L, out, 0L, g, accumulate, scale, out2,
                       nsplit);
  } else {
    hipLaunchKernelGGL(smer_col_reduce, dim3(gx.x, 1), dim3(256), 0, s, nblk, N, part, stride,
                       off, out, 0L, nblk, accumulate, scale, out2, nsplit);
  }
}

extern "C" int smer_wce_denom(int n, const int64_t* y, const float* ce_all, float* denom,
                              smer_stream_t stream) {
  SMER_REQUIRE(y && ce_all && denom, "smer_wce_denom: null pointer");
  hipLaunchKernelGGL(wce_denom_kernel, dim3(1), dim3(256), 0, (hipStream_t)stream, n, y, ce_all,
                     denom);
  SMER_CHECK_LAUNCH("smer_wce_denom");
  return SMER_OK;
}

extern "C" int smer_wce_fwd_bwd(int dtype, int R, int V, const float* logits, long ldl,
                                const int64_t* y, const float* w, const float* denom,
                                float* row_loss, float* loss_out, void* dlogits, long ldd,
                                float grad_scale, smer_stream_t stream) {
  SMER_REQUIRE(logits && y && w && denom && row_loss, "smer_wce_fwd_bwd: null pointer");
  if (R == 0) return SMER_OK;
  hipStream_t s = (hipStream_t)stream;
  dim3 grid((R + 3) / 4);
  if (dtype == SMER_BF16)
    hipLaunchKernelGGL(wce_kernel<bf16>, grid, dim3(256), 0, s, R, V, logits, ldl, y, w, denom,
                       row_loss, (bf16*)dlogits, ldd, grad_scale);
  else if (dtype == SMER_F32)
    hipLaunchKernelGGL(wce_kernel<float>, grid, dim3(256), 0, s, R, V, logits, ldl, y, w, denom,
                       row_loss, (float*)dlogits, ldd, grad_scale);
  else
    return smer_set_error(SMER_ERR_UNSUPPORTED, "smer_wce_fwd_bwd: dtype");
  if (loss_out)
    hipLaunchKernelGGL(sum_div_kernel, dim3(1), dim3(256), 0, s, R, row_loss, denom, loss_out);
  SMER_CHECK_LAUNCH("smer_wce_fwd_bwd");
  return SMER_OK;
}

extern "C" int smer_adam(long n, float* p, const float* g, float* m, float* v, void* p_bf16,
                         float lr, float b1, float b2, float eps, float bc1, float bc2_sqrt,
                         smer_stream_t stream) {
  SMER_REQUIRE(p && g && m && v, "smer_adam: null pointer");
  if (n == 0) return SMER_OK;
  long blocks = (n + 255) / 256;
  if (blocks > 8192) blocks = 8192;
  hipLaunchKernelGGL(adam_kernel, dim3(blocks), dim3(256), 0, (hipStream_t)stream, n, p, g, m, v,
                     (bf16*)p_bf16, lr, b1, b2, eps, bc1, bc2_sqrt);
  SMER_CHECK_LAUNCH("smer_adam");
  return SMER_OK;
}

extern "C" int smer_cast(int src_dtype, int dst_dtype, long n, const void* src, void* dst,
                         smer_stream_t stream) {
  if (n == 0) return SMER_OK;
  long blocks = (n + 255) / 256;
  if (blocks > 8192) blocks = 8192;
  hipStream_t s = (hipStream_t)stream;
  if (src_dtype == SMER_F32 && dst_dtype == SMER_BF16)
    hipLaunchKernelGGL((cast_kernel<float, bf16>), dim3(blocks), dim3(256), 0, s, n,
                       (const float*)src, (bf16*)dst);
  else if (src_dtype == SMER_BF16 && dst_dtype == SMER_F32)
    hipLaunchKernelGGL((cast_kernel<bf16, float>), dim3(blocks), dim3(256), 0, s, n,
// ... 151 lines not shown
```

smer_music_generation_amd/engine.py:

```python
from __future__ import annotations

import math
import os

import torch

from . import ops

_SITE = {"pe_src": 1, "pe_tgt": 2}


def _site(kind, layer, which):
    return 16 + (layer * 16 + which) * 2 + (0 if kind == "enc" else 1)


class _W:
    pass


FP8_FFN2 = os.environ.get("SMER_FP8_FFN2", "1") == "1"
FP8_EMBED = os.environ.get("SMER_FP8_EMBED", "0") == "1"
FP8_H8 = (os.environ.get("SMER_FP8_H8", "1") == "1"
          and os.environ.get("SMER_FP8_Q8_FAST", "1") != "0")


_WGRAD_SIDE_CAP = int(os.environ.get("SMER_WGRAD_SIDE_CAP", "0"))
_WGRAD_FP8_CAP = int(os.environ.get("SMER_WGRAD_FP8_CAP", "192"))
_ATTN_MASK_PREGEN = os.environ.get("SMER_ATTN_MASK_PREGEN", "0") == "1"


class Engine:
    def __init__(self, model):
        self.m = model
        self.d = model.d_model
        self.H = model.nhead
        self.D = self.d // self.H
        self.F = model.dim_feedforward
        self.V = model.vocab_size
        self.Vp = (self.V + 63) // 64 * 64
        self.n_enc = model.num_encoder_layers
        self.n_dec = model.num_decoder_layers
        self._bf16 = None
        self._bf16_version = None
        self._fc_pad = None
        self._wgen = 0
        self._ckv_all = None
        self._side = {}
        self._mstream = {}
        self._fp8 = None

    def act_dtype(self):
        return torch.float32 if self.m.precision == "fp32" else torch.bfloat16

    def _weights_flat(self, dt):
        flat = self.m.flat_parameters()
        if dt == torch.float32:
            return flat
        ver = self._version_key()
        if self._bf16 is None or self._bf16.numel() != flat.numel() or self._bf16_version != ver:
            if self._bf16 is None or self._bf16.numel() != flat.numel():
                self._bf16 = torch.empty(flat.numel(), dtype=torch.bfloat16, device=flat.device)
            ops.cast(flat, self._bf16)
            self._fc_pad = None
            self._bf16_version = ver
            self._wgen += 1
        return self._bf16

    def _version_key(self):
        flat = self.m.flat_parameters()
        return (flat.data_ptr(), flat._version, sum(p._version for p in self.m.parameters()))

    def mark_bf16_fresh(self):
        self._bf16_version = self._version_key()
        self._fc_pad = None
        self._wgen += 1

    def mark_params_updated(self):
        self._bf16_version = None
        self._fc_pad = None
        self._wgen += 1

    def weights(self, dt):
        work = self._weights_flat(dt)
        master = self.m.flat_parameters()
        off = self.m._offsets
        d, F, V = self.d, self.F, self.V

        def wv(name, shape):
            o = off[name]
            return work[o: o + math.prod(shape)].view(shape)

        def mv(name, n):
            o = off[name]
            return master[o: o + n]

        W = _W()
        W.emb = mv("embedding.weight", V * d).view(V, d)
        W.enc, W.dec = [], []
        for i in range(self.n_enc):
            p = "transformer.encoder.layers.%d" % i
            L = _W()
            L.in_w, L.in_b = wv(p + ".self_attn.in_proj_weight", (3 * d, d)), mv(p + ".self_attn.in_proj_bias", 3 * d)
            L.out_w, L.out_b = wv(p + ".self_attn.out_proj.weight", (d, d)), mv(p + ".self_attn.out_proj.bias", d)
            L.l1_w, L.l1_b = wv(p + ".linear1.weight", (F, d)), mv(p + ".linear1.bias", F)
            L.l2_w, L.l2_b = wv(p + ".linear2.weight", (d, F)), mv(p + ".linear2.bias", d)
            L.n1 = (mv(p + ".norm1.weight", d), mv(p + ".norm1.bias", d))
            L.n2 = (mv(p + ".norm2.weight", d), mv(p + ".norm2.bias", d))
            W.enc.append(L)
        W.enc_norm = (mv("transformer.encoder.norm.weight", d), mv("transformer.encoder.norm.bias", d))
        for i in range(self.n_dec):
            p = "transformer.decoder.layers.%d" % i
            L = _W()
            L.sa_w, L.sa_b = wv(p + ".self_attn.in_proj_weight", (3 * d, d)), mv(p + ".self_attn.in_proj_bias", 3 * d)
            L.sa_ow, L.sa_ob = wv(p + ".self_attn.out_proj.weight", (d, d)), mv(p + ".self_attn.out_proj.bias", d)
            ca = wv(p + ".multihead_attn.in_proj_weight", (3 * d, d))
            cb = mv(p + ".multihead_attn.in_proj_bias", 3 * d)
            L.cq_w, L.cq_b, L.ckv_w, L.ckv_b = ca[:d], cb[:d], ca[d:], cb[d:]
            L.ca_ow, L.ca_ob = wv(p + ".multihead_attn.out_proj.weight", (d, d)), mv(p + ".multihead_attn.out_proj.bias", d)
            L.l1_w, L.l1_b = wv(p + ".linear1.weight", (F, d)), mv(p + ".linear1.bias", F)
            L.l2_w, L.l2_b = wv(p + ".linear2.weight", (d, F)), mv(p + ".linear2.bias", d)
            L.n1 = (mv(p + ".norm1.weight", d), mv(p + ".norm1.bias", d))
            L.n2 = (mv(p + ".norm2.weight", d), mv(p + ".norm2.bias", d))
            L.n3 = (mv(p + ".norm3.weight", d), mv(p + ".norm3.bias", d))
            W.dec.append(L)
        W.dec_norm = (mv("transformer.decoder.norm.weight", d), mv("transformer.decoder.norm.bias", d))
        W.fc_w = wv("fc.weight", (V, d))
        W.fc_b = mv("fc.bias", V)
        if self._fc_pad is None or self._fc_pad.dtype != dt or self._fc_pad.device != work.device:
            self._fc_pad = torch.zeros(self.Vp, d, dtype=dt, device=work.device)
        ops.cast(W.fc_w.reshape(-1), self._fc_pad[:V].reshape(-1))
# ... 247 lines not shown
                         drop_mask=amask(("dec", i), T, T), drop_mask_in=bool(pregen), q8=q8)
            y1 = self._lin(f8, o, oq, "dec%d.sao" % i, L.sa_ow, L.sa_ob, residual=y, drop_p=p_tr,
                           seed=sd(_site("dec", i, 1)))
            x1, m1, r1, x1q = self._ln_q(f8, y1, L.n1, dt, "dec%d.ln1" % i)
            qc = self._lin(f8, x1, x1q, "dec%d.cq" % i, L.cq_w, L.cq_b)
            kvc = kvc_all[:, i * 2 * d:(i + 1) * 2 * d]
            oc = torch.empty(B * T, d, dtype=dt, device=dev)
            lsec = torch.empty(B, H, T, device=dev)
            q8, ocq = self._attn_q8(f8, oc, "dec%d.oc" % i, D)
            ops.attn_fwd(qc, kvc[:, :d], kvc[:, d:], oc, lsec, B=B, H=H, Lq=T, Lk=S, D=D, kpm=mkpm,
                         causal=False, scale=scale, drop_p=p_tr, seed=sd(_site("dec", i, 2)),
                         drop_mask=amask(("cross", i), T, S), drop_mask_in=bool(pregen), q8=q8)
            if need_weights:
                ops.attn_weights(qc, kvc[:, :d], lsec, wts[i], B=B, H=H, Lq=T, Lk=S, D=D, kpm=mkpm,
                                 scale=scale)
            y2 = self._lin(f8, oc, ocq, "dec%d.cao" % i, L.ca_ow, L.ca_ob, residual=x1, drop_p=p_tr,
                           seed=sd(_site("dec", i, 3)))
            x2, m2, r2, x2q = self._ln_q(f8, y2, L.n2, dt, "dec%d.ln2" % i)
            h, hq = self._lin(f8, x2, x2q, "dec%d.l1" % i, L.l1_w, L.l1_b, q_site="dec%d.h" % i,
                              q_only=self._ffn2_fp8(f8, B * T, L.l2_w, "dec%d.l2" % i),
                              relu=True, drop_p=p_tr, seed=sd(_site("dec", i, 4)))
            y3 = self._lin(f8, h, hq, "dec%d.l2" % i, L.l2_w, L.l2_b, residual=x2, drop_p=p_tr,
                           seed=sd(_site("dec", i, 5)))
            x3, m3, r3, yq = self._ln_q(f8, y3, L.n3, dt,
                                        "dec%d.ln3" % i if i + 1 < self.n_dec else None)
            if save:
                ctx.dec.append((y, qkv, o, lse, y1, m1, r1, x1, qc, kvc, oc, lsec, y2, m2, r2, x2,
                                h, y3, m3, r3))
                ctx.dec_q.append((yq_in, oq, x1q, ocq, x2q, hq))
            y = x3
        out, mo, ro = self._ln(y, W.dec_norm, dt)
        ctx.dec_last = (y, mo, ro)
        ctx.dec_out = out
        logits = torch.empty(B * T, self.V, device=dev)
        ops.gemm(out, W.fc_w, M=B * T, N=self.V, K=d, out_f32=logits, bias=W.fc_b, dtype=dt)
        return logits, wts, ctx

    def _mask_stream(self, dev):
        ms = self._mstream.get(dev)
        if ms is None:
            ms = self._mstream[dev] = torch.cuda.Stream(device=dev)
        return ms

    def _wgrad_stream(self, dev, dt):
        if dt != torch.bfloat16 or os.environ.get("SMER_WGRAD_OVERLAP", "1") == "0":
            return None
        side = self._side.get(dev)
        if side is None:
            side = (torch.cuda.Stream(device=dev),
                    torch.zeros(ops.SPLITK_WS_BYTES, dtype=torch.uint8, device=dev))
            self._side[dev] = side
        return side

    @staticmethod
    def _wgrad(side, dy, x, gw, q8=None, **kw):
        def run(ws, cap):
            if q8 is not None and ops.linear_wgrad_fp8(q8[0], q8[1], q8[2], q8[3], gw, db=kw.get("db"),
                                                       accumulate=kw.get("accumulate", True), ws=ws,
                                                       max_wg=cap if (_WGRAD_FP8_CAP < 0 or ws is None)
                                                       else _WGRAD_FP8_CAP):
                return
            if x is None or dy is None:
                raise RuntimeError("engine: fp8 weight gradient declined with no bf16 input")
            ops.linear_wgrad(dy, x, gw, ws=ws, max_wg=cap, **kw)
        if side is None:
            run(None, 0)
            return
        stream, ws = side
        stream.wait_stream(torch.cuda.current_stream(side[1].device))
        with torch.cuda.stream(stream):
            run(ws, _WGRAD_SIDE_CAP)
            if ops.CK_LOG is not None:
                ops.ck("S:dW", gw)
                ops.ck("S:db", kw.get("db"))
                ops.ck("S:dy", dy)
                ops.ck("S:x", x)
        for t in (dy, x):
            if t is not None:
                t.record_stream(stream)
        if q8 is not None:
            q8[0].record_stream(stream)
            q8[2].record_stream(stream)

    @staticmethod
    def _join(side):
        if side is not None:
            torch.cuda.current_stream(side[0].device).wait_stream(side[0])

    @staticmethod
    def _hook(side, hook, name):
        if side is None:
            hook(name)
            return
        with torch.cuda.stream(side[0]):
            hook(name)

    def backward(self, ctx, dlog_pad, hook=None):
        m = self.m
        dt = ctx.dt
        dev = dlog_pad.device
        B, S, T = ctx.B, ctx.S, ctx.T
        d, H, D, V = self.d, self.H, self.D, self.V
        scale = 1.0 / math.sqrt(D)
        p_tr = ctx.p_tr
        sd = lambda site: (ctx.seed * 1000003 + site) & 0xFFFFFFFF
        W = self.weights(dt)
        G = self.grad_views()
        Mt, Ms = B * T, B * S

        from .fp8 import FP8_ATTN_DGRAD, FP8_DGRAD, eligible
        f8 = ctx.f8 if FP8_DGRAD else None

        def ln_bwd(g_in, y_, mu, rs, wb, dx_, dxd_, seed_, gw, site):
            kw = dict(dx_drop=dxd_ if p_tr > 0 else None, drop_p=p_tr, seed=seed_, dgamma=gw[0],
                      dbeta=gw[1], param_stream=ps)
            if f8 is None:
                ops.layernorm_bwd(g_in, y_, mu, rs, wb[0], dx_, **kw)
                if ops.CK_LOG is not None:
                    ops.ck("M:ln_in.g", g_in)
                    ops.ck("M:ln_in.y", y_)
                    ops.ck("M:ln_in.mu", mu)
                    ops.ck("M:ln_in.rs", rs)
                return None
            si = f8.site(site)
            q = torch.empty(y_.shape, dtype=torch.uint8, device=dev)
            ops.layernorm_bwd(g_in, y_, mu, rs, wb[0], dx_, q8=q, qs=f8.qs_of(si), amax=f8.amax_of(si), **kw)
            f8.record_bwd(site)
            return (q, si) if site in f8.bwd_ready else None

        def attn_q8(shape, site, parts):
            if f8 is None or not FP8_ATTN_DGRAD:
                return None, None
            si = f8.site(site)
            buf = torch.empty(shape, dtype=torch.uint8, device=dev)
            views = [None if p is None else buf[:, p[0]:p[1]] for p in parts]
            f8.record_bwd(site)
            return (views[0], views[1], views[2], f8.qs_of(si), f8.amax_of(si)), \
                ((buf, si) if site in f8.bwd_ready else None)

        def dgrad(gq, g, wname, w, q_site=None, q_only=False, **epi):
            M = (g if g is not None else gq[0]).shape[0]
            if gq is not None:
                wt = f8.weight_t(wname)
                if wt is not None and eligible(M, w.shape[1], w.shape[0]):
                    out = None if (q_only and q_site is not None and q_site in f8.bwd_ready) else \
                        torch.empty(M, w.shape[1], dtype=dt, device=dev)
                    if q_site is None:
                        if ops.gemm_fp8_ex(gq[0], f8.inv_of(gq[1]), wt[0], wt[1], out, **epi):
                            return out, None
                    else:
                        si = f8.site(q_site)
                        q = torch.empty(M, w.shape[1], dtype=torch.uint8, device=dev)
                        if ops.gemm_fp8_ex(gq[0], f8.inv_of(gq[1]), wt[0], wt[1], out, q8=q,
                                           qs=f8.qs_of(si), amax=f8.amax_of(si), **epi):
                            f8.record_bwd(q_site)
                            return out, ((q, si) if q_site in f8.bwd_ready else None)
            if g is None:
                raise RuntimeError("engine: %s dgrad has only an e4m3 input but did not run fp8" % wname)
            return ops.linear_dgrad(g, w, **epi), None

        side = self._wgrad_stream(dev, dt)
        ps = side[0] if side is not None else None
        wg_ = lambda *a, **kw: self._wgrad(side, *a, **kw)
        from .fp8 import FP8_WGRAD
        f8w = ctx.f8 if FP8_WGRAD else None

        def wg(dy_, x_, gw, dyq=None, xq=None, **kw):
            if f8w is not None and dyq is not None and xq is not None:
                kw["q8"] = (dyq[0], f8w.inv_of(dyq[1]), xq[0], f8w.inv_of(xq[1]))
            wg_(dy_, x_, gw, **kw)
        def ffn2_bwd(dyq, dyd, name, w2, GL, h, hq, q_site, xq1, name1):
            gs = ops.drop_scale(p_tr)
            Mr = (dyd if dyd is not None else dyq[0]).shape[0]
            q_only = (FP8_H8 and f8 is not None and f8w is not None and xq1 is not None
                      and f8.weight_t(name1) is not None and eligible(Mr, w2.shape[0], w2.shape[1]))
            if h is None and not (f8 is not None and f8w is not None and dyq is not None
                                  and f8.weight_t(name) is not None):
                h = self._deq8(hq, ctx.f8)
            wg(dyd, h, GL.l2_w, dyq, hq, db=GL.l2_b)
            if h is not None:
                return dgrad(dyq, dyd, name, w2, q_site=q_site, q_only=q_only, gate=h, gate_scale=gs)
            wt = f8.weight_t(name)
            si = f8.site(q_site)
            M, N = Mr, w2.shape[1]
            out = None if (q_only and q_site in f8.bwd_ready) else torch.empty(M, N, dtype=dt, device=dev)
            q = torch.empty(M, N, dtype=torch.uint8, device=dev)
            if not ops.gemm_fp8_gate8(dyq[0], f8.inv_of(dyq[1]), wt[0], wt[1], hq[0], gs, out, q,
                                      f8.qs_of(si), f8.amax_of(si)):
                raise RuntimeError("engine: %s e4m3-gated dgrad declined its shape" % name)
            f8.record_bwd(q_site)
            return out, ((q, si) if q_site in f8.bwd_ready else None)

        def q_only_grad(xq_, name, w, site, dropped=True):
            M = ctx.B * (ctx.S if name.startswith("enc") else ctx.T)
            return (FP8_H8 and (p_tr > 0 or not dropped) and f8 is not None and f8w is not None and xq_ is not None
                    and site in f8.bwd_ready and f8.weight_t(name) is not None
                    and eligible(M, w.shape[1], w.shape[0]) and w.shape[0] % 256 == 0 and M % 64 == 0)

        def dgrad_in(y_, xq_, name, w, site):
            if p_tr == 0:
                return None
            return None if q_only_grad(xq_, name, w, site) else torch.empty_like(y_)

        ops.ck("M:dlog", dlog_pad)
        wg(dlog_pad, ctx.dec_out, G.fc_w, M=V, db=G.fc_b)
        g_out = ops.linear_dgrad(dlog_pad, W.fc_pad, K=self.Vp)
        ck = ops.ck
        ck("M:g_out", g_out)
        y_last, mo, ro = ctx.dec_last
        dy = torch.empty_like(y_last)
        ops.layernorm_bwd(g_out, y_last, mo, ro, W.dec_norm[0], dy, dgamma=G.dec_norm[0],
                          dbeta=G.dec_norm[1], param_stream=ps)
        ck("M:dy_final", dy)
        if hook:
            self._hook(side, hook, "head")
        cross8 = None
        if f8 is not None and FP8_ATTN_DGRAD and self.n_dec:
            cross8 = (f8.site("b.cross"), torch.empty(Ms, self.n_dec * 2 * d, dtype=torch.uint8, device=dev))
        kv_q_only = (cross8 is not None and FP8_H8 and f8w is not None and "b.cross" in f8.bwd_ready
                     and ctx.memq is not None and f8.weight_t("ckv") is not None
                     and eligible(Ms, d, self.n_dec * 2 * d) and (2 * d) % 256 == 0 and Ms % 64 == 0)
        dkvc_all = None if kv_q_only else torch.empty(Ms, self.n_dec * 2 * d, dtype=dt, device=dev)
        for i in reversed(range(self.n_dec)):
            L, GL = W.dec[i], G.dec[i]
            (y_in, qkv, o, lse, y1, m1, r1, x1, qc, kvc, oc, lsec, y2, m2, r2, x2, h, y3, m3,
             r3) = ctx.dec[i]
            yq_in, oq, x1q, ocq, x2q, hq = ctx.dec_q[i]
            dy3 = torch.empty_like(y3)
            dy3d = dgrad_in(y3, hq, "dec%d.l2" % i, L.l2_w, "b.dec%d.ln3" % i) if p_tr > 0 else dy3
            dy3q = ln_bwd(dy, y3, m3, r3, L.n3, dy3, dy3d, sd(_site("dec", i, 5)), GL.n3, "b.dec%d.ln3" % i)
            ck("M:dec%d.dy3" % i, dy3d)
            dh, dhq = ffn2_bwd(dy3q, dy3d, "dec%d.l2" % i, L.l2_w, GL, h, hq, "b.dec%d.dh" % i, x2q,
                               "dec%d.l1" % i)
            ck("M:dec%d.dh" % i, dh)
            wg(dh, x2, GL.l1_w, dhq, x2q, db=GL.l1_b)
            dx2, _ = dgrad(dhq, dh, "dec%d.l1" % i, L.l1_w, residual=dy3)
            ck("M:dec%d.dx2" % i, dx2)
            dy2 = torch.empty_like(y2)
            dy2d = dgrad_in(y2, ocq, "dec%d.cao" % i, L.ca_ow, "b.dec%d.ln2" % i) if p_tr > 0 else dy2
            dy2q = ln_bwd(dx2, y2, m2, r2, L.n2, dy2, dy2d, sd(_site("dec", i, 3)), GL.n2, "b.dec%d.ln2" % i)
            ck("M:dec%d.dy2" % i, dy2d)
            wg(dy2d, oc, GL.ca_ow, dy2q, ocq, db=GL.ca_ob)
            doc, _ = dgrad(dy2q, dy2d, "dec%d.cao" % i, L.ca_ow)
            ck("M:dec%d.doc" % i, doc)
            dqc = None if (cross8 is not None and q_only_grad(x1q, "dec%d.cq" % i, L.cq_w, "b.cross",
                                                              dropped=False)) else \
                torch.empty(Mt, d, dtype=dt, device=dev)
            dkvc = dkvc_all[:, i * 2 * d:(i + 1) * 2 * d] if dkvc_all is not None else None
            q8c, dqcq = None, None
            if cross8 is not None:
                si, dkvc8 = cross8
                dqc8 = torch.empty(Mt, d, dtype=torch.uint8, device=dev)
                q8c = (dqc8, dkvc8[:, i * 2 * d:i * 2 * d + d], dkvc8[:, i * 2 * d + d:(i + 1) * 2 * d],
                       f8.qs_of(si), f8.amax_of(si))
                f8.record_bwd("b.cross")
                dqcq = (dqc8, si) if "b.cross" in f8.bwd_ready else None
            ops.attn_bwd(qc, kvc[:, :d], kvc[:, d:], oc, doc, lsec, dqc,
                         dkvc[:, :d] if dkvc is not None else None, dkvc[:, d:] if dkvc is not None else None,
                         B=B, H=H, Lq=T, Lk=S, D=D, kpm=ctx.mkpm, causal=False, scale=scale,
                         drop_p=p_tr, seed=sd(_site("dec", i, 2)), drop_mask=ctx.masks.get(("cross", i)),
                         q8=q8c)
            ck("M:dec%d.dqc" % i, dqc)
            ck("M:dec%d.dkvc" % i, dkvc)
            wg(dqc, x1, GL.cq_w, dqcq, x1q, db=GL.cq_b)
            dkvcq = None
            if cross8 is not None and "b.cross" in f8.bwd_ready:
                dkvcq = (cross8[1][:, i * 2 * d:(i + 1) * 2 * d], cross8[0])
            wg(dkvc, ctx.mem, GL.ckv_w, dkvcq, ctx.memq, db=GL.ckv_b)
            dx1, _ = dgrad(dqcq, dqc, "dec%d.cq" % i, L.cq_w, residual=dy2)
            ck("M:dec%d.dx1" % i, dx1)
            dy1 = torch.empty_like(y1)
            dy1d = dgrad_in(y1, oq, "dec%d.sao" % i, L.sa_ow, "b.dec%d.ln1" % i) if p_tr > 0 else dy1
            dy1q = ln_bwd(dx1, y1, m1, r1, L.n1, dy1, dy1d, sd(_site("dec", i, 1)), GL.n1, "b.dec%d.ln1" % i)
            ck("M:dec%d.dy1" % i, dy1d)
            wg(dy1d, o, GL.sa_ow, dy1q, oq, db=GL.sa_ob)
            do, _ = dgrad(dy1q, dy1d, "dec%d.sao" % i, L.sa_ow)
            ck("M:dec%d.do" % i, do)
            q8s, dqkvq = attn_q8((Mt, 3 * d), "b.dec%d.dqkv" % i, [(0, d), (d, 2 * d), (2 * d, 3 * d)])
            dqkv = None if (q8s is not None and q_only_grad(yq_in, "dec%d.sa" % i, L.sa_w, "b.dec%d.dqkv" % i,
                                                            dropped=False)) else \
                torch.empty(Mt, 3 * d, dtype=dt, device=dev)
            dq_, dk_, dv_ = (None, None, None) if dqkv is None else \
                (dqkv[:, :d], dqkv[:, d:2 * d], dqkv[:, 2 * d:])
            ops.attn_bwd(qkv[:, :d], qkv[:, d:2 * d], qkv[:, 2 * d:], o, do, lse, dq_,
                         dk_, dv_, B=B, H=H, Lq=T, Lk=T, D=D,
                         kpm=ctx.tkpm, causal=True, scale=scale, drop_p=p_tr,
                         seed=sd(_site("dec", i, 0)), drop_mask=ctx.masks.get(("dec", i)), q8=q8s)
            ck("M:dec%d.dqkv" % i, dqkv)
            wg(dqkv, y_in, GL.sa_w, dqkvq, yq_in, db=GL.sa_b)
            dy, _ = dgrad(dqkvq, dqkv, "dec%d.sa" % i, L.sa_w, residual=dy1)
            ck("M:dec%d.dy" % i, dy)
            if hook:
                self._hook(side, hook, "dec%d" % i)
        d_tgt = dy
        if self.n_dec:
            if kv_q_only or (cross8 is not None and "b.cross" in f8.bwd_ready and f8.weight_t("ckv") is not None
                             and eligible(Ms, d, self.n_dec * 2 * d)):
                dmem, _ = dgrad((cross8[1], cross8[0]), dkvc_all, "ckv", W.ckv_all)
            else:
                dmem = ops.linear_dgrad(dkvc_all, W.ckv_all, out_f32=torch.empty(Ms, d, device=dev))
        else:
            dmem = torch.zeros(Ms, d, device=dev)
        ck("M:dmem", dmem)
        x_last, me, re = ctx.enc_last
        dx = torch.empty_like(x_last)
        ops.layernorm_bwd(dmem, x_last, me, re, W.enc_norm[0], dx, dgamma=G.enc_norm[0],
                          dbeta=G.enc_norm[1], param_stream=ps)
        for i in reversed(range(self.n_enc)):
            L, GL = W.enc[i], G.enc[i]
            (x_in, qkv, o, lse, y1, m1, r1, x1, h, y2, m2, r2) = ctx.enc[i]
            xq_in, oq, x1q, hq = ctx.enc_q[i]
            dy2 = torch.empty_like(y2)
            dy2d = dgrad_in(y2, hq, "enc%d.l2" % i, L.l2_w, "b.enc%d.ln2" % i) if p_tr > 0 else dy2
            dy2q = ln_bwd(dx, y2, m2, r2, L.n2, dy2, dy2d, sd(_site("enc", i, 3)), GL.n2, "b.enc%d.ln2" % i)
            ck("M:enc%d.dy2" % i, dy2d)
            dh, dhq = ffn2_bwd(dy2q, dy2d, "enc%d.l2" % i, L.l2_w, GL, h, hq, "b.enc%d.dh" % i, x1q,
                               "enc%d.l1" % i)
            ck("M:enc%d.dh" % i, dh)
            wg(dh, x1, GL.l1_w, dhq, x1q, db=GL.l1_b)
            dx1, _ = dgrad(dhq, dh, "enc%d.l1" % i, L.l1_w, residual=dy2)
            ck("M:enc%d.dx1" % i, dx1)
            dy1 = torch.empty_like(y1)
            dy1d = dgrad_in(y1, oq, "enc%d.out" % i, L.out_w, "b.enc%d.ln1" % i) if p_tr > 0 else dy1
            dy1q = ln_bwd(dx1, y1, m1, r1, L.n1, dy1, dy1d, sd(_site("enc", i, 1)), GL.n1, "b.enc%d.ln1" % i)
            ck("M:enc%d.dy1" % i, dy1d)
            wg(dy1d, o, GL.out_w, dy1q, oq, db=GL.out_b)
            do, _ = dgrad(dy1q, dy1d, "enc%d.out" % i, L.out_w)
            ck("M:enc%d.do" % i, do)
            q8s, dqkvq = attn_q8((Ms, 3 * d), "b.enc%d.dqkv" % i, [(0, d), (d, 2 * d), (2 * d, 3 * d)])
            dqkv = None if (q8s is not None and q_only_grad(xq_in, "enc%d.in" % i, L.in_w, "b.enc%d.dqkv" % i,
                                                            dropped=False)) else \
                torch.empty(Ms, 3 * d, dtype=dt, device=dev)
            dq_, dk_, dv_ = (None, None, None) if dqkv is None else \
                (dqkv[:, :d], dqkv[:, d:2 * d], dqkv[:, 2 * d:])
            ops.attn_bwd(qkv[:, :d], qkv[:, d:2 * d], qkv[:, 2 * d:], o, do, lse, dq_,
                         dk_, dv_, B=B, H=H, Lq=S, Lk=S, D=D,
                         kpm=ctx.skpm, causal=False, scale=scale, drop_p=p_tr,
                         seed=sd(_site("enc", i, 0)), drop_mask=ctx.masks.get(("enc", i)), q8=q8s)
            ck("M:enc%d.dqkv" % i, dqkv)
            wg(dqkv, x_in, GL.in_w, dqkvq, xq_in, db=GL.in_b)
            dx, _ = dgrad(dqkvq, dqkv, "enc%d.in" % i, L.in_w, residual=dy1)
            ck("M:enc%d.dx" % i, dx)
            if hook:
                self._hook(side, hook, "enc%d" % i)
        ops.embed_bwd(G.emb, math.sqrt(d), [(ctx.src_ids, dx, ctx.p_pos, sd(_SITE["pe_src"])),
                                            (ctx.tgt_ids, d_tgt, ctx.p_pos, sd(_SITE["pe_tgt"]))])
        self._join(side)
        if hook:
            hook("embedding")


class ScoreTransformerFunction(torch.autograd.Function):
    @staticmethod
    def forward(fctx, anchor, model, need_grad, src, tgt, src_kpm, tgt_kpm, mem_kpm, tgt_mask):
        eng = model.engine
        if not src.is_cuda:
            raise RuntimeError("the SMER engine runs on the GPU: move the model and inputs to "
                               "a ROCm device first")
        training = model.training and (model.pos_dropout > 0 or model.trans_dropout > 0)
        seed = int(torch.randint(0, 2 ** 31 - 1, (1,)).item()) if training else 0
        logits, wts, ctx = eng.forward(src, tgt, src_kpm, tgt_kpm, mem_kpm,
                                       training=model.training, need_weights=model.need_weights,
                                       save=need_grad, seed=seed)
        fctx.eng = eng
        fctx.ctx = ctx
        fctx.model = model
        B, T = tgt.shape
        out = logits.view(B, T, eng.V)
        w = wts.permute(1, 0, 2, 3) if wts is not None else None
        if w is not None:
            fctx.mark_non_differentiable(w)
        return out, w

    @staticmethod
    def backward(fctx, dlogits, dweights):
        eng = fctx.eng
        ctx = fctx.ctx
        B, T = ctx.B, ctx.T
        dl = torch.zeros(B * T, eng.Vp, dtype=ctx.dt, device=dlogits.device)
        ops.cast2d(dlogits.reshape(B * T, eng.V).contiguous().float(), dl, cols=eng.V)
        eng.backward(ctx, dl)
        fctx.ctx = None
        return (None,) * 9
```

smer_music_generation_amd/ops.py:

```python
from __future__ import annotations

import torch

from ._lib import call, load

F32, BF16 = 0, 1


def dtype_code(t: torch.dtype) -> int:
    if t == torch.float32:
        return F32
    if t == torch.bfloat16:
        return BF16
    raise TypeError("unsupported dtype %s" % t)


def _p(t):
    if t is None:
        return None
    if not t.is_cuda:
        raise RuntimeError("smer op: tensor must be on the GPU (got %s)" % t.device)
    return t.data_ptr()


# ... 36 lines not shown


GEMM_TIMER = None


def gemm(A, B, *, M, N, K, a_kcontig=True, b_kcontig=True, out=None, out_f32=None,
         accumulate=False, bias=None, alpha=1.0, relu=False, residual=None, gate=None,
         gate_scale=1.0, drop_p=0.0, seed=0, dtype=None):
    dt = dtype_code(dtype if dtype is not None else A.dtype)
    timer = GEMM_TIMER
    if timer is not None:
        ev0 = torch.cuda.Event(enable_timing=True)
        ev1 = torch.cuda.Event(enable_timing=True)
        ev0.record()
    _gemm_call(dt, A, B, M, N, K, a_kcontig, b_kcontig, out, out_f32, accumulate, bias, alpha,
               relu, residual, gate, gate_scale, drop_p, seed)
    if timer is not None:
        ev1.record()
        epi = "".join(c for c, on in (("b", bias is not None), ("r", relu), ("d", drop_p > 0),
                                      ("R", residual is not None), ("g", gate is not None),
                                      ("f", out_f32 is not None), ("+", accumulate)) if on)
        tag = "%s%s M%d N%d K%d %s" % ("n" if a_kcontig else "t", "t" if b_kcontig else "n",
                                        M, N, K, epi)
        timer.records.append((ev0, ev1, 2.0 * M * N * K, tag))


class CkLog:

    PARTS = 64

    def __init__(self, device, n=4096, keep=()):
        self.buf = torch.zeros(n * self.PARTS, dtype=torch.int64, device=device)
        self.n = n
        self.names = []
        self.keep = tuple(keep)
        self.kept = {}

    def add(self, name, t):
        i = len(self.names)
        if i >= self.n:
            return
        if t.dim() == 1:
            rows, row_b, ld_b = 1, t.numel() * t.element_size(), t.numel() * t.element_size()
        else:
            t2 = t.reshape(-1, t.shape[-1]) if t.dim() > 2 else t
            rows, row_b, ld_b = t2.shape[0], t2.shape[1] * t2.element_size(), _ld(t2) * t2.element_size()
        self.names.append((name, torch.cuda.current_stream(t.device).cuda_stream))
        call("smer_debug_checksum", _p(t), rows, row_b, ld_b, self.buf.data_ptr() + i * self.PARTS * 8,
             self.PARTS, _stream())
        if any(k in name for k in self.keep):
            self.kept[i] = t.clone()

    def values(self):
        import numpy as np
        v = self.buf.view(self.n, self.PARTS)[:len(self.names)].cpu().numpy().view(np.uint64)
        return [int(x) for x in v.sum(axis=1, dtype=np.uint64)]

    def reset(self):
        self.buf.zero_()
        self.names = []
        self.kept = {}


CK_LOG = None


def ck(name, t):
    if CK_LOG is not None and t is not None:
        CK_LOG.add(name, t)


_SPLITK_WS = {}
SPLITK_WS_BYTES = 64 << 20


def splitk_workspace(device):
    ws = _SPLITK_WS.get(device)
    if ws is None:
        ws = torch.zeros(SPLITK_WS_BYTES, dtype=torch.uint8, device=device)
        _SPLITK_WS[device] = ws
    return ws


def _gemm_call(dt, A, B, M, N, K, a_kcontig, b_kcontig, out, out_f32, accumulate, bias, alpha,
               relu, residual, gate, gate_scale, drop_p, seed):
    ws = None
    if out_f32 is not None and out is None and bias is None and residual is None and gate is None:
        ws = splitk_workspace(A.device)
    call("smer_gemm", dt, int(a_kcontig), int(b_kcontig), M, N, K, _p(A), _ld(A), _p(B), _ld(B),
         _p(bias), float(alpha), int(relu), _p(residual),
         _ld(residual) if residual is not None else 0, _p(gate),
         _ld(gate) if gate is not None else 0, float(gate_scale), float(drop_p),
         int(seed) & 0xFFFFFFFF, _p(out), _ld(out) if out is not None else 0, _p(out_f32),
         _ld(out_f32) if out_f32 is not None else 0, int(accumulate), _p(ws),
         ws.numel() if ws is not None else 0, _stream())


def linear(x, w, bias=None, *, out=None, out_f32=None, accumulate=False, relu=False,
           residual=None, drop_p=0.0, seed=0):
    M, K = x.shape
    N = w.shape[0]
    if out is None and out_f32 is None:
        out = torch.empty(M, N, device=x.device, dtype=x.dtype)
    gemm(x, w, M=M, N=N, K=K, out=out, out_f32=out_f32, accumulate=accumulate, bias=bias,
         relu=relu, residual=residual, drop_p=drop_p, seed=seed, dtype=x.dtype)
    return out if out is not None else out_f32


def linear_dgrad(dy, w, *, K=None, out=None, residual=None, gate=None, gate_scale=1.0,
                 out_f32=None, accumulate=False):
    M = dy.shape[0]
    Kc = K if K is not None else w.shape[0]
    Nin = w.shape[1]
    if out is None and out_f32 is None:
        out = torch.empty(M, Nin, device=dy.device, dtype=dy.dtype)
    gemm(dy, w, M=M, N=Nin, K=Kc, a_kcontig=True, b_kcontig=False, out=out, out_f32=out_f32,
         accumulate=accumulate, residual=residual, gate=gate, gate_scale=gate_scale,
         dtype=dy.dtype)
    return out if out is not None else out_f32


def linear_wgrad(dy, x, dw, *, M=None, accumulate=True, db=None, ws=None, max_wg=0):
    T = dy.shape[0]
    Mo = M if M is not None else dy.shape[1]
    if db is not None and dy.dtype == torch.bfloat16:
        if ws is None:
            ws = splitk_workspace(dy.device)
        timer = GEMM_TIMER
        if timer is not None:
            ev0 = torch.cuda.Event(enable_timing=True)
            ev1 = torch.cuda.Event(enable_timing=True)
            ev0.record()
        call("smer_gemm_wgrad_bias_ex", BF16, Mo, x.shape[1], T, _p(dy), _ld(dy), _p(x), _ld(x),
             _p(dw), _ld(dw), int(accumulate), _p(db), int(accumulate), _p(ws), ws.numel(),
             int(max_wg), _stream())
        if timer is not None:
            ev1.record()
            timer.records.append((ev0, ev1, 2.0 * Mo * x.shape[1] * T,
                                  "wgrad+bias M%d N%d K%d" % (Mo, x.shape[1], T)))
        return
    gemm(dy, x, M=Mo, N=x.shape[1], K=T, a_kcontig=False, b_kcontig=False, out_f32=dw,
         accumulate=accumulate, dtype=dy.dtype)
    if db is not None:
        colsum(dy, db, N=Mo, accumulate=accumulate)


def attn_drop_mask(B, H, Lq, Lk, device):
    n = load().smer_attn_drop_mask_bytes(B, H, Lq, Lk)
    return torch.empty(max(16, n), dtype=torch.uint8, device=device)


_WARNED_P = set()


def attn_drop_rate(p):
    if p <= 0:
        return 0.0
    return min(127, max(1, int(p * 128.0 + 0.5))) / 128.0


def _check_attn_p(p):
    r = attn_drop_rate(p)
    if p > 0 and abs(r - p) > 0.1 * p and p not in _WARNED_P:
        import warnings
        _WARNED_P.add(p)
        warnings.warn("attention dropout p=%g is realised as %g (1/128 granularity of the "
                      "attention kernels); activation dropout sites keep p to 1/65536" % (p, r))


def attn_fwd(q, k, v, o, lse, *, B, H, Lq, Lk, D, kpm=None, causal=False, scale, drop_p=0.0,
             seed=0, drop_mask=None, drop_mask_in=False, q8=None):
    _check_attn_p(drop_p)
    if q8 is not None:
        if dtype_code(q.dtype) != BF16:
            raise RuntimeError("attn_fwd: the e4m3 copy needs bf16")
        o8, qs, amax = q8
        call("smer_attn_fwd_fp8", B, H, Lq, Lk, D, _p(q), _ld(q), _p(k), _ld(k), _p(v), _ld(v), _p(o),
             _ld(o), _p(lse), _p(kpm), int(causal), float(scale), float(drop_p), int(seed) & 0xFFFFFFFF,
             _p(drop_mask), int(bool(drop_mask_in)), _p(o8), _ld(o8), _p(qs), _p(amax), _stream())
        return
    call("smer_attn_fwd", dtype_code(q.dtype), B, H, Lq, Lk, D, _p(q), _ld(q), _p(k), _ld(k),
         _p(v), _ld(v), _p(o), _ld(o), _p(lse), _p(kpm), int(causal), float(scale),
         float(drop_p), int(seed) & 0xFFFFFFFF, _p(drop_mask), int(bool(drop_mask_in)), _stream())


def attn_drop_mask_gen(mask, *, B, H, Lq, Lk, drop_p, seed):
    call("smer_attn_drop_mask_gen", B, H, Lq, Lk, float(drop_p), int(seed) & 0xFFFFFFFF,
         _p(mask), _stream())


def attn_bwd(q, k, v, o, do, lse, dq, dk, dv, *, B, H, Lq, Lk, D, kpm=None, causal=False,
             scale, drop_p=0.0, seed=0, drop_mask=None, q8=None):
    lib = load()
    dt = dtype_code(q.dtype)
    nbytes = lib.smer_attn_bwd_workspace(dt, B, H, Lq, Lk)
    ws = torch.empty(max(1, nbytes), dtype=torch.uint8, device=q.device)
    if q8 is not None:
        if dt != BF16:
            raise RuntimeError("attn_bwd: e4m3 copies need bf16")
        dq8, dk8, dv8, qs, amax = q8
        ld8 = lambda t: _ld(t) if t is not None else 0
        call("smer_attn_bwd_fp8", B, H, Lq, Lk, D, _p(q), _ld(q), _p(k), _ld(k), _p(v), _ld(v),
             _p(o), _ld(o), _p(do), _ld(do), _p(lse), _p(kpm), int(causal), float(scale),
             float(drop_p), int(seed) & 0xFFFFFFFF, _p(dq), ld8(dq), _p(dk), ld8(dk), _p(dv),
             ld8(dv), _p(ws), nbytes, _p(drop_mask), _p(dq8), ld8(dq8), _p(dk8), ld8(dk8),
             _p(dv8), ld8(dv8), _p(qs), _p(amax), _stream())
        return
    call("smer_attn_bwd", dt, B, H, Lq, Lk, D, _p(q), _ld(q), _p(k), _ld(k), _p(v), _ld(v),
         _p(o), _ld(o), _p(do), _ld(do), _p(lse), _p(kpm), int(causal), float(scale),
         float(drop_p), int(seed) & 0xFFFFFFFF, _p(dq), _ld(dq), _p(dk), _ld(dk), _p(dv),
         _ld(dv), _p(ws), nbytes, _p(drop_mask), _stream())


def attn_weights(q, k, lse, out, *, B, H, Lq, Lk, D, kpm=None, causal=False, scale):
    call("smer_attn_weights", dtype_code(q.dtype), B, H, Lq, Lk, D, _p(q), _ld(q), _p(k),
         _ld(k), _p(lse), _p(kpm), int(causal), float(scale), _p(out), _stream())


# ... 261 lines not shown
                  (meta, torch.int32), (out_tok, torch.int32), (alive, torch.int32)):
        if t.dtype != dt or not t.is_contiguous():
            raise RuntimeError("grammar_greedy_step: expected contiguous %s" % dt)
    if logits.shape[0] < 2 * R or ids.shape[0] != 2 * R or meta.shape != (4, 2 * R) or \
            targets.shape[0] != R or keep.shape[0] != 13 or cls.shape[0] != V or src_len.shape[0] != R:
        raise RuntimeError("grammar_greedy_step: shape mismatch")
    if ring is not None:
        if ring.dtype != torch.int32 or not ring.is_pinned() or alive.numel() < 3:
            raise RuntimeError("grammar_greedy_step: ring must be pinned int32, alive int32 [3]")
        call("smer_grammar_greedy_step_ring", R, V, _p(logits), _ld(logits), _p(state), nst,
             _p(targets), targets.shape[1], _p(keep), _p(cls), int(eos), int(m0), int(trash_pos),
             int(max_span), _p(src_len), _p(ids), _p(meta), _p(out_tok), out_tok.shape[1],
             _p(alive), ring.data_ptr(), ring.numel(), _stream())
        return
    call("smer_grammar_greedy_step", R, V, _p(logits), _ld(logits), _p(state), nst, _p(targets),
         targets.shape[1], _p(keep), _p(cls), int(eos), int(m0), int(trash_pos), int(max_span),
         _p(src_len), _p(ids), _p(meta), _p(out_tok), out_tok.shape[1], _p(alive), _stream())


def grammar_sample_step(logits, state, targets, keep, reject, cls, src_len, ids, meta, out_tok, mt,
                        ctl, *, eos, m0, trash_pos, max_span=100, ring=None, tp=None):
    R, nst = state.shape
    V = keep.shape[1]
    for t, dt in ((state, torch.int32), (targets, torch.int8), (keep, torch.uint8),
                  (reject, torch.uint8), (cls, torch.uint8), (src_len, torch.int32),
                  (ids, torch.int64), (meta, torch.int32), (out_tok, torch.int32),
                  (mt, torch.int32), (ctl, torch.int32)):
        if t.dtype != dt or not t.is_contiguous():
            raise RuntimeError("grammar_sample_step: expected contiguous %s" % dt)
    if logits.shape[0] < 2 * R or ids.shape[0] != 2 * R or meta.shape != (4, 2 * R) or \
            targets.shape[0] != R or keep.shape[0] != 13 or reject.shape != keep.shape or \
            cls.shape[0] != V or src_len.shape[0] != R or mt.numel() < 625 or ctl.numel() < 3:
        raise RuntimeError("grammar_sample_step: shape mismatch")
    if ring is not None and (ring.dtype != torch.int32 or not ring.is_pinned()):
        raise RuntimeError("grammar_sample_step: ring must be pinned int32")
    args = (R, V, _p(logits), _ld(logits), _p(state), nst, _p(targets),
            targets.shape[1], _p(keep), _p(reject), _p(cls), int(eos), int(m0), int(trash_pos),
            int(max_span), _p(src_len), _p(ids), _p(meta), _p(out_tok), out_tok.shape[1], _p(mt),
            _p(ctl), ring.data_ptr() if ring is not None else None, ring.numel() if ring is not None else 0)
    if tp is None:
        call("smer_grammar_sample_step", *args, _stream())
        return
    if tp.dtype != torch.float64 or not tp.is_contiguous() or tuple(tp.shape) != (R, 2) or \
            tp.device != state.device:
        raise RuntimeError("grammar_sample_step: tp must be contiguous float64 [R, 2] on the device")
    call("smer_grammar_sample_step_tp", *args, _p(tp), _stream())


def grammar_sample_step_rows(logits, state, targets, keep, reject, cls, src_len, ids, meta, out_tok,
                             mt, ctl, *, eos, m0, trash_pos, max_span=100, ring=None, tp=None):
    R, nst = state.shape
    V = keep.shape[1]
    for t, dt in ((state, torch.int32), (targets, torch.int8), (keep, torch.uint8),
                  (reject, torch.uint8), (cls, torch.uint8), (src_len, torch.int32),
                  (ids, torch.int64), (meta, torch.int32), (out_tok, torch.int32),
                  (mt, torch.int32), (ctl, torch.int32)):
        if t.dtype != dt or not t.is_contiguous():
            raise RuntimeError("grammar_sample_step_rows: expected contiguous %s" % dt)
    if logits.shape[0] < 2 * R or ids.shape[0] != 2 * R or meta.shape != (4, 2 * R) or \
            targets.shape[0] != R or keep.shape[0] != 13 or reject.shape != keep.shape or \
            cls.shape[0] != V or src_len.shape[0] != R or mt.dim() != 2 or mt.shape[0] != R or \
            mt.shape[1] < 625 or ctl.numel() < 3 or out_tok.shape[0] != R:
        raise RuntimeError("grammar_sample_step_rows: shape mismatch")
    if ring is not None and (ring.dtype != torch.int32 or not ring.is_pinned()):
        raise RuntimeError("grammar_sample_step_rows: ring must be pinned int32")
    if tp is not None and (tp.dtype != torch.float64 or not tp.is_contiguous() or
                           tuple(tp.shape) != (R, 2) or tp.device != state.device):
        raise RuntimeError("grammar_sample_step_rows: tp must be contiguous float64 [R, 2] on the device")
    call("smer_grammar_sample_step_rows", R, V, _p(logits), _ld(logits), _p(state), nst, _p(targets),
         targets.shape[1], _p(keep), _p(reject), _p(cls), int(eos), int(m0), int(trash_pos),
         int(max_span), _p(src_len), _p(ids), _p(meta), _p(out_tok), out_tok.shape[1], _p(mt),
         mt.shape[1], _p(ctl), ring.data_ptr() if ring is not None else None,
         ring.numel() if ring is not None else 0, _p(tp), _stream())


def layernorm(x, gamma, beta, y, mean, rstd, eps=1e-5):
    M, N = x.shape
    call("smer_layernorm_fwd", dtype_code(x.dtype), M, N, _p(x), _ld(x), _p(gamma), _p(beta),
         float(eps), _p(y), _ld(y), _p(mean), _p(rstd), _stream())


def layernorm_bwd(dy, x, mean, rstd, gamma, dx, *, dx_drop=None, drop_p=0.0, seed=0,
                  dgamma=None, dbeta=None, accumulate=True, param_stream=None, q8=None, qs=None,
                  amax=None):
    lib = load()
    M, N = x.shape
    nbytes = lib.smer_layernorm_bwd_workspace(M, N) if (dgamma is not None or dbeta is not None) else 0
    ws = torch.empty(max(1, nbytes), dtype=torch.uint8, device=x.device)
    if q8 is not None:
        if x.dtype != torch.bfloat16 or dy.dtype != torch.bfloat16:
            raise RuntimeError("layernorm_bwd: the e4m3 copy needs bf16 dy and x")
        partial = param_stream is not None and nbytes > 0
        call("smer_layernorm_bwd_fp8", M, N, _p(dy), _ld(dy), _p(x), _ld(x), _p(mean), _p(rstd),
             _p(gamma), _p(dx), _ld(dx), _p(dx_drop), _ld(dx_drop) if dx_drop is not None else 0,
             float(drop_p), int(seed) & 0xFFFFFFFF, _p(q8), _ld(q8), _p(qs), _p(amax),
             _p(None if partial else dgamma), _p(None if partial else dbeta), int(accumulate),
             _p(ws), nbytes, int(partial), _stream())
        if partial:
            param_stream.wait_stream(torch.cuda.current_stream(x.device))
            with torch.cuda.stream(param_stream):
                call("smer_layernorm_param_reduce", M, N, _p(ws), nbytes, _p(dgamma), _p(dbeta),
                     int(accumulate), _stream())
            ws.record_stream(param_stream)
        return
    if param_stream is not None and nbytes:
        call("smer_layernorm_bwd_partials", dtype_code(x.dtype), M, N, _p(dy), _ld(dy),
             int(dy.dtype == torch.float32 and x.dtype != torch.float32), _p(x), _ld(x), _p(mean),
             _p(rstd), _p(gamma), _p(dx), _ld(dx), _p(dx_drop),
             _ld(dx_drop) if dx_drop is not None else 0, float(drop_p), int(seed) & 0xFFFFFFFF,
             _p(ws), nbytes, _stream())
        param_stream.wait_stream(torch.cuda.current_stream(x.device))
        with torch.cuda.stream(param_stream):
            call("smer_layernorm_param_reduce", M, N, _p(ws), nbytes, _p(dgamma), _p(dbeta),
                 int(accumulate), _stream())
        ws.record_stream(param_stream)
        return
    call("smer_layernorm_bwd", dtype_code(x.dtype), M, N, _p(dy), _ld(dy),
         int(dy.dtype == torch.float32 and x.dtype != torch.float32), _p(x), _ld(x), _p(mean),
         _p(rstd), _p(gamma), _p(dx), _ld(dx), _p(dx_drop),
         _ld(dx_drop) if dx_drop is not None else 0, float(drop_p), int(seed) & 0xFFFFFFFF,
         _p(dgamma), _p(dbeta), int(accumulate), _p(ws), nbytes, _stream())


def embed(ids, table, pe, out, *, L=0, positions=None, scale, drop_p=0.0, seed=0):
    n_tok = ids.numel()
    d = table.shape[1]
    call("smer_embed_fwd", dtype_code(out.dtype), n_tok, d, _p(ids), _p(positions), int(L),
         _p(table), _p(pe), float(scale), float(drop_p), int(seed) & 0xFFFFFFFF, _p(out),
         _ld(out), _stream())


def embed_fp8(ids, table, pe, out, q8, qs, amax, *, L=0, positions=None, scale, drop_p=0.0, seed=0):
    n_tok = ids.numel()
    d = table.shape[1]
    call("smer_embed_fwd_fp8", n_tok, d, _p(ids), _p(positions), int(L), _p(table), _p(pe), float(scale),
         float(drop_p), int(seed) & 0xFFFFFFFF, _p(out), _ld(out), _p(q8), _ld(q8), _p(qs), _p(amax), _stream())


def embed_bwd(dtable, scale, segs):
    lib = load()
    V, d = dtable.shape
    segs = list(segs) + [(None, None, 0.0, 0)] * (2 - len(segs))
    (i0, x0, p0, s0), (i1, x1, p1, s1) = segs
    n0 = i0.numel() if i0 is not None else 0
    n1 = i1.numel() if i1 is not None else 0
    dt = dtype_code((x0 if x0 is not None else x1).dtype)
    nbytes = lib.smer_embed_bwd_workspace(V, d, n0 + n1)
    ws = torch.empty(max(1, nbytes), dtype=torch.uint8, device=dtable.device)
    call("smer_embed_bwd", dt, V, d, float(scale), _p(i0), _p(x0),
         _ld(x0) if x0 is not None else 0, n0, float(p0), int(s0) & 0xFFFFFFFF, _p(i1), _p(x1),
         _ld(x1) if x1 is not None else 0, n1, float(p1), int(s1) & 0xFFFFFFFF, _p(dtable),
         _p(ws), nbytes, _stream())


def wce_denom(y, ce_all, denom):
    call("smer_wce_denom", y.numel(), _p(y), _p(ce_all), _p(denom), _stream())


def wce_fwd_bwd(logits, y, w, denom, row_loss, loss_out=None, dlogits=None, *, V=None,
                grad_scale=1.0):
    R = logits.shape[0]
    Vv = V if V is not None else logits.shape[1]
    dt = dtype_code(dlogits.dtype) if dlogits is not None else F32
    call("smer_wce_fwd_bwd", dt, R, Vv, _p(logits), _ld(logits), _p(y), _p(w), _p(denom),
         _p(row_loss), _p(loss_out), _p(dlogits), _ld(dlogits) if dlogits is not None else 0,
         float(grad_scale), _stream())


def argmax_accuracy(logits, y, cls, ncls, pad, counts):
    R, V = logits.shape
    if y.dtype != torch.int64 or cls.dtype != torch.int32 or counts.dtype != torch.int32:
        raise TypeError("argmax_accuracy: int64 targets, int32 class table and counts")
    if counts.numel() < 2 * ncls + 2:
        raise ValueError("argmax_accuracy: counts needs 2 * ncls + 2 entries")
    call("smer_argmax_accuracy", R, V, _p(logits), _ld(logits), _p(y), _p(cls), int(ncls), int(pad),
         _p(counts), _stream())


def adam(p, g, m, v, p_bf16, *, lr, b1, b2, eps, step):
    import math
    bc1 = 1.0 - b1 ** step
    bc2s = math.sqrt(1.0 - b2 ** step)
    call("smer_adam", p.numel(), _p(p), _p(g), _p(m), _p(v), _p(p_bf16), float(lr), float(b1),
         float(b2), float(eps), float(bc1), float(bc2s), _stream())


def cast(src, dst):
    assert src.numel() == dst.numel()
    call("smer_cast", dtype_code(src.dtype), dtype_code(dst.dtype), src.numel(), _p(src),
         _p(dst), _stream())


def cast2d(src, dst, *, rows=None, cols=None):
    r = rows if rows is not None else src.shape[0]
    c = cols if cols is not None else src.shape[1]
    call("smer_cast2d", dtype_code(src.dtype), dtype_code(dst.dtype), r, c, _p(src), _ld(src),
         _p(dst), _ld(dst), _stream())
# ... 11 lines not shown
```

Baseline: 3.132 million train tokens/s (B*(S+T)).

## Batch split-K and layernorm parameter reductions into one per-layer queued kernel

Adds a gradient-reduce queue that defers the split-K weight-gradient reduce kernels and the layernorm gamma/beta column reductions. Each layer's reductions then run as a single batched kernel on the side stream, found through a job table and a binary search. The goal is to cut kernel launch count and per-launch overhead in the backward pass. The cost is a host-to-device table copy per flush, an event sync on slot reuse, a dedicated workspace that may regrow with a device sync, and a wider ABI.

```diff
diff --git a/include/smer_hip.h b/include/smer_hip.h
--- a/include/smer_hip.h
+++ b/include/smer_hip.h
@@ -37,7 +37,13 @@
 int smer_gemm_wgrad_bias_ex(int dtype, int M, int N, int K, const void* dy, long lddy,
                             const void* x, long ldx, float* dW, long lddw, int accumulate,
                             float* db, int db_accumulate, void* workspace, size_t ws_bytes,
-                            int max_workgroups, smer_stream_t stream);
+                            int max_workgroups, void* queue, smer_stream_t stream);
+int smer_grad_queue_create(size_t ws_bytes, void** queue);
+int smer_grad_queue_destroy(void* queue);
+size_t smer_grad_queue_workspace_bytes(int n);
+int smer_grad_reduce_begin(void* queue);
+int smer_grad_reduce_flush(void* queue, smer_stream_t stream);
+int smer_grad_queue_stats(void* queue, long* counters);
 int smer_gemm_wgrad_fp8(int M, int N, int K, const void* dy8, long lddy, const void* x8, long ldx,
                         const float* dy_inv, const float* x_inv, float* dW, long lddw, int accumulate,
                         float* db, int db_accumulate, void* workspace, size_t ws_bytes,
@@ -186,7 +192,7 @@
                                 long ldxd, float drop_p, uint32_t seed, void* workspace,
                                 size_t ws_bytes, smer_stream_t stream);
 int smer_layernorm_param_reduce(int M, int N, void* workspace, size_t ws_bytes, float* dgamma,
-                                float* dbeta, int accumulate, smer_stream_t stream);
+                                float* dbeta, int accumulate, void* queue, smer_stream_t stream);
 
 int smer_embed_fwd(int dtype, int n_tok, int d, const int64_t* ids, const int32_t* positions,
                    int L, const float* table, const float* pe, float scale,
diff --git a/smer_music_generation_amd/_lib.py b/smer_music_generation_amd/_lib.py
--- a/smer_music_generation_amd/_lib.py
+++ b/smer_music_generation_amd/_lib.py
@@ -26,7 +26,13 @@
     "smer_gemm_wgrad_fp8": (c_int, [c_int, c_int, c_int, P, c_long, P, c_long, P, P, P, c_long, c_int, P, c_int,
                                     P, c_size, c_int, P]),
     "smer_gemm_wgrad_bias_ex": (c_int, [c_int, c_int, c_int, c_int, P, c_long, P, c_long, P, c_long,
-                                        c_int, P, c_int, P, c_size, c_int, P]),
+                                        c_int, P, c_int, P, c_size, c_int, P, P]),
+    "smer_grad_queue_create": (c_int, [c_size, ctypes.POINTER(ctypes.c_void_p)]),
+    "smer_grad_queue_destroy": (c_int, [P]),
+    "smer_grad_queue_workspace_bytes": (c_size, [c_int]),
+    "smer_grad_reduce_begin": (c_int, [P]),
+    "smer_grad_reduce_flush": (c_int, [P, P]),
+    "smer_grad_queue_stats": (c_int, [P, ctypes.POINTER(ctypes.c_long)]),
     "smer_attn_fwd": (c_int, [c_int, c_int, c_int, c_int, c_int, c_int, P, c_long, P, c_long, P,
                               c_long, P, c_long, P, P, c_int, c_float, c_float, c_u32, P, c_int, P]),
     "smer_attn_fwd_fp8": (c_int, [c_int, c_int, c_int, c_int, c_int, P, c_long, P, c_long, P, c_long,
@@ -112,7 +118,7 @@
                                    c_long, P, c_long, c_float, c_u32, P, P, c_int, P, c_size, P]),
     "smer_layernorm_bwd_partials": (c_int, [c_int, c_int, c_int, P, c_long, c_int, P, c_long, P, P,
                                             P, P, c_long, P, c_long, c_float, c_u32, P, c_size, P]),
-    "smer_layernorm_param_reduce": (c_int, [c_int, c_int, P, c_size, P, P, c_int, P]),
+    "smer_layernorm_param_reduce": (c_int, [c_int, c_int, P, c_size, P, P, c_int, P, P]),
     "smer_embed_fwd": (c_int, [c_int, c_int, c_int, P, P, c_int, P, P, c_float, c_float, c_u32,
                                P, c_long, P]),
     "smer_embed_bwd_workspace": (c_size, [c_int, c_int, c_int]),
diff --git a/smer_music_generation_amd/csrc/common.h b/smer_music_generation_amd/csrc/common.h
--- a/smer_music_generation_amd/csrc/common.h
+++ b/smer_music_generation_amd/csrc/common.h
@@ -117,6 +117,27 @@
                             int accumulate, float scale, float* scratch, hipStream_t s,
                             float* out2 = nullptr, int nsplit = 0);
 
+template <typename LD>
+__device__ __forceinline__ float col_reduce_rows(int b0, int b1, int g, LD ld) {
+  float a0 = 0.f, a1 = 0.f, a2 = 0.f, a3 = 0.f;
+  int b = b0 + g;
+  for (; b + 12 < b1; b += 16) {
+    a0 += ld(b);
+    a1 += ld(b + 4);
+    a2 += ld(b + 8);
+    a3 += ld(b + 12);
+  }
+  for (; b < b1; b += 4) a0 += ld(b);
+  return (a0 + a1) + (a2 + a3);
+}
+__device__ __forceinline__ float col_reduce_join(const float (*red)[64], int cl) {
+  return (red[0][cl] + red[1][cl]) + (red[2][cl] + red[3][cl]);
+}
+
+int smer_grad_queue_push_col(void* queue, int nblk, int N, const float* part, long stride, long off,
+                             float* out, int accumulate, float scale, float* out2, int nsplit,
+                             hipStream_t s);
+
 template <typename T, bool VEC = true>
 __device__ __forceinline__ void load8(const T* p, int valid, float (&v)[8]) {
   if (VEC && valid >= 8) {
diff --git a/smer_music_generation_amd/csrc/gemm.hip b/smer_music_generation_amd/csrc/gemm.hip
--- a/smer_music_generation_amd/csrc/gemm.hip
+++ b/smer_music_generation_amd/csrc/gemm.hip
@@ -1801,14 +1801,15 @@
   }
 }
 
-__global__ void splitk_reduce_kernel(int M, int N, int ksplit, const float* __restrict__ slabs,
-                                     float alpha, float* __restrict__ Cf, long ldcf,
-                                     int accumulate, const float* __restrict__ rs_part,
-                                     float* __restrict__ rs_out, int rs_accumulate) {
-  long idx = ((long)blockIdx.x * blockDim.x + threadIdx.x) * 4;
+__device__ __forceinline__ void splitk_reduce_item(long gtid, int M, int N, int ksplit,
+                                                   const float* __restrict__ slabs, float alpha,
+                                                   float* __restrict__ Cf, long ldcf, int accumulate,
+                                                   const float* __restrict__ rs_part,
+                                                   float* __restrict__ rs_out, int rs_accumulate) {
+  long idx = gtid * 4;
   long MN = (long)M * N;
   if (idx >= MN) {
-    const long m = ((long)blockIdx.x * blockDim.x + threadIdx.x) - MN / 4;
+    const long m = gtid - MN / 4;
     if (rs_out == nullptr || m >= M) return;
     float t = 0.f;
     for (int s = 0; s < ksplit; ++s) t += rs_part[(long)s * M + m];
@@ -1848,6 +1849,96 @@
     int row = e / N, col = e % N;
     float* p = Cf + (long)row * ldcf + col;
     *p = accumulate ? *p + v[t] : v[t];
+  }
+}
+
+__global__ void splitk_reduce_kernel(int M, int N, int ksplit, const float* __restrict__ slabs,
+                                     float alpha, float* __restrict__ Cf, long ldcf,
+                                     int accumulate, const float* __restrict__ rs_part,
+                                     float* __restrict__ rs_out, int rs_accumulate) {
+  splitk_reduce_item((long)blockIdx.x * blockDim.x + threadIdx.x, M, N, ksplit, slabs, alpha, Cf, ldcf,
+                     accumulate, rs_part, rs_out, rs_accumulate);
+}
+
+constexpr int GRQ_MAX_JOBS = 32;
+constexpr int GRQ_SLOTS = 32;
+constexpr int GRQ_COL_CHUNKS = 64;
+struct GradReduceJob {
+  int kind;
+  int M, N;
+  int split;
+  const float* src;
+  const float* rs_part;
+  float* out;
+  float* out2;
+  long ld, off;
+  float alpha;
+  int accumulate, rs_accumulate;
+  int block0;
+};
+
+__global__ __launch_bounds__(256) void grad_reduce_batch_kernel(const GradReduceJob* __restrict__ jobs,
+                                                                int njobs) {
+  __shared__ float red[2][4][64];
+  __shared__ float lvl1[GRQ_COL_CHUNKS][64];
+  int lo = 0, hi = njobs - 1;
+  while (lo < hi) {
+    const int mid = (lo + hi + 1) >> 1;
+    if (jobs[mid].block0 <= (int)blockIdx.x) lo = mid;
+    else hi = mid - 1;
+  }
+  const GradReduceJob j = jobs[lo];
+  const int lb = blockIdx.x - j.block0;
+  if (j.kind == 0) {
+    splitk_reduce_item((long)lb * 256 + threadIdx.x, j.M, j.N, j.split, j.src, j.alpha, j.out, j.ld,
+                       j.accumulate, j.rs_part, j.out2, j.rs_accumulate);
+    return;
+  }
+  const int nblk = j.M, N = j.N;
+  const int cl = threadIdx.x & 63, g = threadIdx.x >> 6;
+  const int col = lb * 64 + cl;
+  const bool ok = col < N;
+  const float* p = j.src + j.off + (ok ? col : 0);
+  const long stride = j.ld;
+  auto ldp = [&](int b) { return p[(long)b * stride]; };
+  float a;
+  if (nblk <= 64) {
+    red[0][g][cl] = ok ? col_reduce_rows(0, nblk, g, ldp) : 0.f;
+    __syncthreads();
+    a = col_reduce_join(red[0], cl);
+  } else {
+    const int nch = (nblk + 63) / 64;
+    for (int y = 0; y < nch; y += 2) {
+      const int b0 = y * 64;
+      float s0 = 0.f, s1 = 0.f;
+      if (ok) {
+        if (b0 + 128 <= nblk) {
+          float v[2][16];
+#pragma unroll
+          for (int c = 0; c < 2; ++c)
+#pragma unroll
+            for (int i = 0; i < 16; ++i) v[c][i] = p[(long)(b0 + 64 * c + g + 4 * i) * stride];
+          s0 = col_reduce_rows(0, 64, 0, [&](int b) { return v[0][b >> 2]; });
+          s1 = col_reduce_rows(0, 64, 0, [&](int b) { return v[1][b >> 2]; });
+        } else {
+          s0 = col_reduce_rows(b0, min(nblk, b0 + 64), g, ldp);
+          if (y + 1 < nch) s1 = col_reduce_rows(b0 + 64, min(nblk, b0 + 128), g, ldp);
+        }
+      }
+      red[0][g][cl] = s0;
+      red[1][g][cl] = s1;
+      __syncthreads();
+      if (g < 2 && y + g < nch) lvl1[y + g][cl] = col_reduce_join(red[g], cl);
+      __syncthreads();
+    }
+    red[0][g][cl] = col_reduce_rows(0, nch, g, [&](int b) { return lvl1[b][cl]; });
+    __syncthreads();
+    a = col_reduce_join(red[0], cl);
+  }
+  if (g == 0 && ok) {
+    a *= j.alpha;
+    float* o = col < j.split ? j.out + col : j.out2 + (col - j.split);
+    *o = j.accumulate ? *o + a : a;
   }
 }
 
@@ -2071,6 +2162,149 @@
   s = std::min<long>(s, (long)(splitk_slab_bytes(ws_bytes) / (((size_t)M * N + M) * sizeof(float))));
   s = std::max<long>(1, std::min<long>(s, 64));
   return (int)s;
+}
+
+struct GradQueue {
+  int dev = 0;
+  char* ws = nullptr;
+  size_t ws_bytes = 0, used = 0;
+  GradReduceJob* host_tab = nullptr;
+  GradReduceJob* dev_tab = nullptr;
+  hipEvent_t slot_done[GRQ_SLOTS] = {};
+  int slot = 0, njobs = 0, nblocks = 0;
+  long flushes = 0, launches = 0;
+  GradReduceJob jobs[GRQ_MAX_JOBS];
+};
+static thread_local GradQueue* g_grad_queue = nullptr;
+static thread_local bool g_grad_queue_failed = false;
+
+static int grad_queue_flush(GradQueue* q, hipStream_t s) {
+  if (q->njobs == 0) {
+    q->used = 0;
+    return SMER_OK;
+  }
+  const int k = q->slot;
+  if (hipEventSynchronize(q->slot_done[k]) != hipSuccess)
+    return smer_set_error(SMER_ERR_HIP, "smer_grad_reduce_flush: event");
+  GradReduceJob* h = q->host_tab + (size_t)k * GRQ_MAX_JOBS;
+  GradReduceJob* d = q->dev_tab + (size_t)k * GRQ_MAX_JOBS;
+  for (int i = 0; i < q->njobs; ++i) h[i] = q->jobs[i];
+  if (hipMemcpyAsync(d, h, sizeof(GradReduceJob) * q->njobs, hipMemcpyHostToDevice, s) != hipSuccess)
+    return smer_set_error(SMER_ERR_HIP, "smer_grad_reduce_flush: table copy");
+  hipLaunchKernelGGL(grad_reduce_batch_kernel, dim3(q->nblocks), dim3(256), 0, s,
+                     (const GradReduceJob*)d, q->njobs);
+  hipEventRecord(q->slot_done[k], s);
+  q->slot = (k + 1) % GRQ_SLOTS;
+  q->njobs = 0;
+  q->nblocks = 0;
+  q->used = 0;
+  q->flushes++;
+  q->launches++;
+  SMER_CHECK_LAUNCH("smer_grad_reduce_flush");
+  return SMER_OK;
+}
+
+static int grad_queue_push(GradQueue* q, const GradReduceJob& job, int blocks, hipStream_t s) {
+  if (q->njobs == GRQ_MAX_JOBS) {
+    const size_t keep = q->used;
+    int rc = grad_queue_flush(q, s);
+    if (rc != SMER_OK) return rc;
+    q->used = keep;
+  }
+  GradReduceJob& j = q->jobs[q->njobs++];
+  j = job;
+  j.block0 = q->nblocks;
+  q->nblocks += blocks;
+  return SMER_OK;
+}
+
+static void* grad_queue_alloc(GradQueue* q, size_t bytes, hipStream_t s) {
+  bytes = (bytes + 255) & ~(size_t)255;
+  if (q->used + bytes > q->ws_bytes) {
+    if (grad_queue_flush(q, s) != SMER_OK) return nullptr;
+    if (bytes > q->ws_bytes) {
+      if (hipDeviceSynchronize() != hipSuccess) return nullptr;
+      if (q->ws) hipFree(q->ws);
+      q->ws = nullptr;
+      q->ws_bytes = 0;
+      if (hipMalloc((void**)&q->ws, bytes) != hipSuccess) return nullptr;
+      q->ws_bytes = bytes;
+    }
+  }
+  void* p = q->ws + q->used;
+  q->used += bytes;
+  return p;
+}
+
+int smer_grad_queue_push_col(void* queue, int nblk, int N, const float* part, long stride, long off,
+                             float* out, int accumulate, float scale, float* out2, int nsplit,
+                             hipStream_t s) {
+  GradQueue* q = (GradQueue*)queue;
+  if (nblk > 64 * GRQ_COL_CHUNKS) return SMER_ERR_UNSUPPORTED;
+  GradReduceJob j{};
+  j.kind = 1; j.M = nblk; j.N = N; j.split = out2 ? nsplit : N;
+  j.src = part; j.ld = stride; j.off = off; j.out = out; j.out2 = out2;
+  j.alpha = scale; j.accumulate = accumulate;
+  return grad_queue_push(q, j, (N + 63) / 64, s);
+}
+
+extern "C" int smer_grad_queue_create(size_t ws_bytes, void** queue) {
+  SMER_REQUIRE(queue, "smer_grad_queue_create: null pointer");
+  GradQueue* q = new GradQueue();
+  bool ok = hipGetDevice(&q->dev) == hipSuccess;
+  q->ws_bytes = (std::max<size_t>(ws_bytes, 256) + 255) & ~(size_t)255;
+  ok = ok && hipMalloc((void**)&q->ws, q->ws_bytes) == hipSuccess;
+  const size_t tab = sizeof(GradReduceJob) * GRQ_SLOTS * GRQ_MAX_JOBS;
+  ok = ok && hipHostMalloc((void**)&q->host_tab, tab, hipHostMallocDefault) == hipSuccess;
+  ok = ok && hipMalloc((void**)&q->dev_tab, tab) == hipSuccess;
+  for (int i = 0; ok && i < GRQ_SLOTS; ++i)
+    ok = hipEventCreateWithFlags(&q->slot_done[i], hipEventDisableTiming) == hipSuccess;
+  if (!ok) {
+    (void)hipGetLastError();
+    smer_grad_queue_destroy(q);
+    return smer_set_error(SMER_ERR_HIP, "smer_grad_queue_create: allocation failed");
+  }
+  *queue = q;
+  return SMER_OK;
+}
+
+extern "C" int smer_grad_queue_destroy(void* queue) {
+  GradQueue* q = (GradQueue*)queue;
+  if (!q) return SMER_OK;
+  if (q->ws) hipFree(q->ws);
+  if (q->dev_tab) hipFree(q->dev_tab);
+  if (q->host_tab) hipHostFree(q->host_tab);
+  for (int i = 0; i < GRQ_SLOTS; ++i)
+    if (q->slot_done[i]) hipEventDestroy(q->slot_done[i]);
+  delete q;
+  return SMER_OK;
+}
+
+extern "C" size_t smer_grad_queue_workspace_bytes(int n) {
+  g_wgrad_cap = 0;
+  return (size_t)std::max(1, n) * (size_t)smer_wgrad_resident() * (GBM * GBN + GBM) * sizeof(float);
+}
+
+extern "C" int smer_grad_reduce_begin(void* queue) {
+  GradQueue* q = (GradQueue*)queue;
+  SMER_REQUIRE(q, "smer_grad_reduce_begin: null queue");
+  q->njobs = 0;
+  q->nblocks = 0;
+  q->used = 0;
+  return SMER_OK;
+}
+
+extern "C" int smer_grad_reduce_flush(void* queue, smer_stream_t stream) {
+  SMER_REQUIRE(queue, "smer_grad_reduce_flush: null queue");
+  return grad_queue_flush((GradQueue*)queue, (hipStream_t)stream);
+}
+
+extern "C" int smer_grad_queue_stats(void* queue, long* counters) {
+  GradQueue* q = (GradQueue*)queue;
+  SMER_REQUIRE(q && counters, "smer_grad_queue_stats: null pointer");
+  counters[0] = q->njobs; counters[1] = (long)q->used; counters[2] = q->flushes;
+  counters[3] = (long)q->ws_bytes;
+  return SMER_OK;
 }
 
 static bool smer_skinny_kf() {
@@ -2217,6 +2451,14 @@
     kchunk = ((K + split - 1) / split + GBK - 1) / GBK * GBK;
     split = (K + kchunk - 1) / kchunk;
   }
+  GradQueue* gq = (split > 1 && !smer_splitk_fused()) ? g_grad_queue : nullptr;
+  if (gq) {
+    ws = grad_queue_alloc(gq, ((size_t)split * M * N + (size_t)split * M) * sizeof(float), s);
+    if (!ws) {
+      g_grad_queue_failed = true;
+      return;
+    }
+  }
   float* rs_part = (split > 1 && rowsum) ? (float*)ws + (size_t)split * M * N : nullptr;
   unsigned* tickets = nullptr;
   if (split > 1 && smer_splitk_fused() && (N & 3) == 0 && (e.ldcf & 3) == 0 &&
@@ -2269,6 +2511,14 @@
 reduce:
   if (split > 1 && !tickets) {
     long n4 = ((long)M * N) / 4 + (rowsum ? M : 0);
+    if (gq) {
+      GradReduceJob j{};
+      j.M = M; j.N = N; j.split = split; j.src = (const float*)ws; j.rs_part = rs_part;
+      j.out = e.Cf; j.out2 = rowsum; j.ld = e.ldcf; j.alpha = e.alpha;
+      j.accumulate = e.accumulate; j.rs_accumulate = e.rs_accumulate;
+      if (grad_queue_push(gq, j, (int)((n4 + 255) / 256), s) != SMER_OK) g_grad_queue_failed = true;
+      return;
+    }
     hipLaunchKernelGGL(splitk_reduce_kernel, dim3((n4 + 255) / 256), dim3(256), 0, s, M, N, split,
                        (const float*)ws, e.alpha, e.Cf, e.ldcf, e.accumulate,
                        (const float*)rs_part, rowsum, e.rs_accumulate);
@@ -2512,13 +2762,14 @@
                                     float* db, int db_accumulate, void* workspace,
                                     size_t ws_bytes, smer_stream_t stream) {
   return smer_gemm_wgrad_bias_ex(dtype, M, N, K, dy, lddy, x, ldx, dW, lddw, accumulate, db,
-                                 db_accumulate, workspace, ws_bytes, 0, stream);
+                                 db_accumulate, workspace, ws_bytes, 0, nullptr, stream);
 }
 
 extern "C" int smer_gemm_wgrad_bias_ex(int dtype, int M, int N, int K, const void* dy, long lddy,
                                        const void* x, long ldx, float* dW, long lddw, int accumulate,
                                        float* db, int db_accumulate, void* workspace,
-                                       size_t ws_bytes, int max_workgroups, smer_stream_t stream) {
+                                       size_t ws_bytes, int max_workgroups, void* queue,
+                                       smer_stream_t stream) {
   SMER_REQUIRE(dtype == SMER_BF16, "smer_gemm_wgrad_bias: bf16 only (fp32: smer_gemm + smer_colsum)");
   SMER_REQUIRE(M > 0 && N > 0 && K > 0, "smer_gemm_wgrad_bias: bad sizes");
   SMER_REQUIRE(dy && x && dW && db, "smer_gemm_wgrad_bias: null pointer");
@@ -2533,8 +2784,12 @@
   auto a16 = [](const void* p, long ld) { return p == nullptr || ((((uintptr_t)p) & 15) == 0 && ld % 8 == 0); };
   e.vec = a16(dW, lddw);
   g_wgrad_cap = max_workgroups > 0 ? max_workgroups : 0;
+  g_grad_queue = (GradQueue*)queue;
+  g_grad_queue_failed = false;
   launch_bf16<false, false>(M, N, K, dy, lddy, x, ldx, e, workspace, ws_bytes, (hipStream_t)stream, db);
   g_wgrad_cap = 0;
+  g_grad_queue = nullptr;
+  if (g_grad_queue_failed) return smer_set_error(SMER_ERR_HIP, "smer_gemm_wgrad_bias: gradient-reduce queue");
   SMER_CHECK_LAUNCH("smer_gemm_wgrad_bias");
   return SMER_OK;
 }
diff --git a/smer_music_generation_amd/csrc/norm_embed.hip b/smer_music_generation_amd/csrc/norm_embed.hip
--- a/smer_music_generation_amd/csrc/norm_embed.hip
+++ b/smer_music_generation_amd/csrc/norm_embed.hip
@@ -916,13 +916,23 @@
 
 extern "C" int smer_layernorm_param_reduce(int M, int N, void* workspace, size_t ws_bytes,
                                            float* dgamma, float* dbeta, int accumulate,
-                                           smer_stream_t stream) {
+                                           void* queue, smer_stream_t stream) {
   SMER_REQUIRE(workspace && ws_bytes >= smer_layernorm_bwd_workspace(M, N),
                "smer_layernorm_param_reduce: workspace too small");
   if (M == 0 || (!dgamma && !dbeta)) return SMER_OK;
   const int nblk = (M + ln_bwd_rows(M, N) - 1) / ln_bwd_rows(M, N);
   float* part = (float*)workspace;
   hipStream_t s = (hipStream_t)stream;
+  if (queue) {
+    int rc;
+    if (dgamma && dbeta)
+      rc = smer_grad_queue_push_col(queue, nblk, 2 * N, part, (long)2 * N, 0L, dgamma, accumulate, 1.f, dbeta, N, s);
+    else if (dgamma)
+      rc = smer_grad_queue_push_col(queue, nblk, N, part, (long)2 * N, 0L, dgamma, accumulate, 1.f, nullptr, 0, s);
+    else
+      rc = smer_grad_queue_push_col(queue, nblk, N, part, (long)2 * N, (long)N, dbeta, accumulate, 1.f, nullptr, 0, s);
+    if (rc != SMER_ERR_UNSUPPORTED) return rc;
+  }
   if (dgamma && dbeta)
     smer_col_reduce_launch(nblk, 2 * N, part, (long)2 * N, 0L, dgamma, accumulate, 1.f,
                            part + (size_t)nblk * 2 * N, s, dbeta, N);
diff --git a/smer_music_generation_amd/csrc/train_ops.hip b/smer_music_generation_amd/csrc/train_ops.hip
--- a/smer_music_generation_amd/csrc/train_ops.hip
+++ b/smer_music_generation_amd/csrc/train_ops.hip
@@ -136,22 +136,15 @@
   const int cl = threadIdx.x & 63, g = threadIdx.x >> 6;
   const int col = blockIdx.x * 64 + cl;
   const int b0 = blockIdx.y * chunk, b1 = min(nblk, b0 + chunk);
-  float a0 = 0.f, a1 = 0.f, a2 = 0.f, a3 = 0.f;
+  float a = 0.f;
   if (col < N) {
     const float* p = part + off + col;
-    int b = b0 + g;
-    for (; b + 12 < b1; b += 16) {
-      a0 += p[(long)b * stride];
-      a1 += p[(long)(b + 4) * stride];
-      a2 += p[(long)(b + 8) * stride];
-      a3 += p[(long)(b + 12) * stride];
-    }
-    for (; b < b1; b += 4) a0 += p[(long)b * stride];
-  }
-  red[g][cl] = (a0 + a1) + (a2 + a3);
+    a = col_reduce_rows(b0, b1, g, [&](int b) { return p[(long)b * stride]; });
+  }
+  red[g][cl] = a;
   __syncthreads();
   if (g == 0 && col < N) {
-    float a = ((red[0][cl] + red[1][cl]) + (red[2][cl] + red[3][cl])) * scale;
+    float a = col_reduce_join(red, cl) * scale;
     float* o = col < nsplit ? out + (long)blockIdx.y * ostride + col
                             : out2 + (long)blockIdx.y * ostride + (col - nsplit);
     *o = accumulate ? *o + a : a;
diff --git a/smer_music_generation_amd/engine.py b/smer_music_generation_amd/engine.py
--- a/smer_music_generation_amd/engine.py
+++ b/smer_music_generation_amd/engine.py
@@ -46,6 +46,7 @@
         self._wgen = 0
         self._ckv_all = None
         self._side = {}
+        self._gqueue = {}
         self._mstream = {}
         self._fp8 = None
 
@@ -459,6 +460,21 @@
             q8[0].record_stream(stream)
             q8[2].record_stream(stream)
 
+    def _grad_queue(self, side):
+        if side is None or ops.CK_LOG is not None or os.environ.get("SMER_GRAD_REDUCE_BATCH", "1") == "0":
+            return None
+        dev = side[1].device
+        gq = self._gqueue.get(dev)
+        if gq is None:
+            gq = self._gqueue[dev] = ops.GradReduceQueue(dev)
+        return gq
+
+    @staticmethod
+    def _flush(side, gq):
+        if gq is not None:
+            with torch.cuda.stream(side[0]):
+                gq.flush()
+
     @staticmethod
     def _join(side):
         if side is not None:
@@ -490,7 +506,7 @@
 
         def ln_bwd(g_in, y_, mu, rs, wb, dx_, dxd_, seed_, gw, site):
             kw = dict(dx_drop=dxd_ if p_tr > 0 else None, drop_p=p_tr, seed=seed_, dgamma=gw[0],
-                      dbeta=gw[1], param_stream=ps)
+                      dbeta=gw[1], param_stream=ps, queue=gq)
             if f8 is None:
                 ops.layernorm_bwd(g_in, y_, mu, rs, wb[0], dx_, **kw)
                 if ops.CK_LOG is not None:
@@ -538,7 +554,10 @@
 
         side = self._wgrad_stream(dev, dt)
         ps = side[0] if side is not None else None
-        wg_ = lambda *a, **kw: self._wgrad(side, *a, **kw)
+        gq = self._grad_queue(side)
+        if gq is not None:
+            gq.begin()
+        wg_ = lambda *a, **kw: self._wgrad(side, *a, queue=gq, **kw)
         from .fp8 import FP8_WGRAD
         f8w = ctx.f8 if FP8_WGRAD else None
 
@@ -587,8 +606,9 @@
         y_last, mo, ro = ctx.dec_last
         dy = torch.empty_like(y_last)
         ops.layernorm_bwd(g_out, y_last, mo, ro, W.dec_norm[0], dy, dgamma=G.dec_norm[0],
-                          dbeta=G.dec_norm[1], param_stream=ps)
+                          dbeta=G.dec_norm[1], param_stream=ps, queue=gq)
         ck("M:dy_final", dy)
+        self._flush(side, gq)
         if hook:
             self._hook(side, hook, "head")
         cross8 = None
@@ -667,6 +687,7 @@
             wg(dqkv, y_in, GL.sa_w, dqkvq, yq_in, db=GL.sa_b)
             dy, _ = dgrad(dqkvq, dqkv, "dec%d.sa" % i, L.sa_w, residual=dy1)
             ck("M:dec%d.dy" % i, dy)
+            self._flush(side, gq)
             if hook:
                 self._hook(side, hook, "dec%d" % i)
         d_tgt = dy
@@ -682,7 +703,7 @@
         x_last, me, re = ctx.enc_last
         dx = torch.empty_like(x_last)
         ops.layernorm_bwd(dmem, x_last, me, re, W.enc_norm[0], dx, dgamma=G.enc_norm[0],
-                          dbeta=G.enc_norm[1], param_stream=ps)
+                          dbeta=G.enc_norm[1], param_stream=ps, queue=gq)
         for i in reversed(range(self.n_enc)):
             L, GL = W.enc[i], G.enc[i]
             (x_in, qkv, o, lse, y1, m1, r1, x1, h, y2, m2, r2) = ctx.enc[i]
@@ -718,10 +739,12 @@
             wg(dqkv, x_in, GL.in_w, dqkvq, xq_in, db=GL.in_b)
             dx, _ = dgrad(dqkvq, dqkv, "enc%d.in" % i, L.in_w, residual=dy1)
             ck("M:enc%d.dx" % i, dx)
+            self._flush(side, gq)
             if hook:
                 self._hook(side, hook, "enc%d" % i)
         ops.embed_bwd(G.emb, math.sqrt(d), [(ctx.src_ids, dx, ctx.p_pos, sd(_SITE["pe_src"])),
                                             (ctx.tgt_ids, d_tgt, ctx.p_pos, sd(_SITE["pe_tgt"]))])
+        self._flush(side, gq)
         self._join(side)
         if hook:
             hook("embedding")
diff --git a/smer_music_generation_amd/ops.py b/smer_music_generation_amd/ops.py
--- a/smer_music_generation_amd/ops.py
+++ b/smer_music_generation_amd/ops.py
@@ -142,6 +142,55 @@
     return ws
 
 
+class GradReduceQueue:
+
+    LAYER_WGRADS = 7
+
+    def __init__(self, device, ws_bytes=None):
+        import ctypes
+        lib = load()
+        self.device = torch.device(device)
+        if ws_bytes is None:
+            ws_bytes = lib.smer_grad_queue_workspace_bytes(self.LAYER_WGRADS)
+        h = ctypes.c_void_p()
+        with torch.cuda.device(self.device):
+            call("smer_grad_queue_create", int(ws_bytes), ctypes.byref(h))
+        self.handle = h
+        self._held = []
+
+    def begin(self):
+        call("smer_grad_reduce_begin", self.handle)
+        self._held = []
+
+    def hold(self, t):
+        self._held.append(t)
+
+    def flush(self):
+        call("smer_grad_reduce_flush", self.handle, _stream())
+        s = torch.cuda.current_stream(self.device)
+        for t in self._held:
+            t.record_stream(s)
+        self._held = []
+
+    def stats(self):
+        import ctypes
+        c = (ctypes.c_long * 4)()
+        call("smer_grad_queue_stats", self.handle, c)
+        return tuple(c)
+
+    def __del__(self):
+        try:
+            if self.handle:
+                load().smer_grad_queue_destroy(self.handle)
+                self.handle = None
+        except Exception:
+            pass
+
+
+def _q(queue):
+    return queue.handle if queue is not None else None
+
+
 def _gemm_call(dt, A, B, M, N, K, a_kcontig, b_kcontig, out, out_f32, accumulate, bias, alpha,
                relu, residual, gate, gate_scale, drop_p, seed):
     ws = None
@@ -180,7 +229,7 @@
     return out if out is not None else out_f32
 
 
-def linear_wgrad(dy, x, dw, *, M=None, accumulate=True, db=None, ws=None, max_wg=0):
+def linear_wgrad(dy, x, dw, *, M=None, accumulate=True, db=None, ws=None, max_wg=0, queue=None):
     T = dy.shape[0]
     Mo = M if M is not None else dy.shape[1]
     if db is not None and dy.dtype == torch.bfloat16:
@@ -188,12 +237,13 @@
             ws = splitk_workspace(dy.device)
         timer = GEMM_TIMER
         if timer is not None:
+            queue = None
             ev0 = torch.cuda.Event(enable_timing=True)
             ev1 = torch.cuda.Event(enable_timing=True)
             ev0.record()
         call("smer_gemm_wgrad_bias_ex", BF16, Mo, x.shape[1], T, _p(dy), _ld(dy), _p(x), _ld(x),
              _p(dw), _ld(dw), int(accumulate), _p(db), int(accumulate), _p(ws), ws.numel(),
-             int(max_wg), _stream())
+             int(max_wg), _q(queue), _stream())
         if timer is not None:
             ev1.record()
             timer.records.append((ev0, ev1, 2.0 * Mo * x.shape[1] * T,
@@ -621,7 +671,7 @@
 
 def layernorm_bwd(dy, x, mean, rstd, gamma, dx, *, dx_drop=None, drop_p=0.0, seed=0,
                   dgamma=None, dbeta=None, accumulate=True, param_stream=None, q8=None, qs=None,
-                  amax=None):
+                  amax=None, queue=None):
     lib = load()
     M, N = x.shape
     nbytes = lib.smer_layernorm_bwd_workspace(M, N) if (dgamma is not None or dbeta is not None) else 0
@@ -639,7 +689,9 @@
             param_stream.wait_stream(torch.cuda.current_stream(x.device))
             with torch.cuda.stream(param_stream):
                 call("smer_layernorm_param_reduce", M, N, _p(ws), nbytes, _p(dgamma), _p(dbeta),
-                     int(accumulate), _stream())
+                     int(accumulate), _q(queue), _stream())
+            if queue is not None:
+                queue.hold(ws)
             ws.record_stream(param_stream)
         return
     if param_stream is not None and nbytes:
@@ -651,7 +703,9 @@
         param_stream.wait_stream(torch.cuda.current_stream(x.device))
         with torch.cuda.stream(param_stream):
             call("smer_layernorm_param_reduce", M, N, _p(ws), nbytes, _p(dgamma), _p(dbeta),
-                 int(accumulate), _stream())
+                 int(accumulate), _q(queue), _stream())
+        if queue is not None:
+            queue.hold(ws)
         ws.record_stream(param_stream)
         return
     call("smer_layernorm_bwd", dtype_code(x.dtype), M, N, _p(dy), _ld(dy),
```

Measured after the change: 3.133 million train tokens/s (B*(S+T)) (median of 4 runs). No clear change (+0.0%).
